# DakeQQ/Automatic-Speech-Recognition-ASR-ONNX

Measured on AMD Instinct MI355X. Metric: audio-sec/s, SenseVoiceSmall, 8 s @ 16 kHz chunks, batch 64 per GPU (RTF = 1/value per GPU-stream), higher is better.
Workload: dtype bf16; 1 GPU; SenseVoiceSmall bf16 (234 M params, 70 SANM blocks), batch=64 x 8 s per GPU, greedy CTC; step k's audio is resident in HBM when the step starts, batch k+1's host->device copy (pinned, copy stream) and every token-id download are inside the timed region; global_batch=64, parallelism=dp1 (utterance sharding, RCCL arena broadcast + hypothesis gather)

## Files before the change

### automatic-speech-recognition-asr-onnx_amd/_probe.py

```python
from __future__ import annotations

import ctypes as C
import os

import numpy as np

from . import _lib

PROBE_PATH = os.path.join(os.path.dirname(os.path.abspath(__file__)), "libasr_mi355x_probe.so")
_fp, _ip = C.POINTER(C.c_float), C.POINTER(C.c_int32)


class GemmDesc(C.Structure):
    _fields_ = [("M", C.c_int32), ("N", C.c_int32), ("K", C.c_int32), ("a", _fp), ("w", _fp), ("bias", _fp), ("add", _fp),
                ("act", C.c_int32), ("ln", C.c_int32), ("ln_eps", C.c_float), ("argmax", C.c_int32), ("n_valid", C.c_int32),
                ("variant", C.c_int32), ("out_lo", _fp), ("out_f32", _fp), ("out_stats", _fp), ("out_ids", _ip),
                ("kernel", C.c_char * 32)]


class DecodeAttnDesc(C.Structure):
    _fields_ = [("bf16", C.c_int32), ("cross", C.c_int32), ("B", C.c_int32), ("b0", C.c_int32), ("nb", C.c_int32), ("H", C.c_int32),
                ("n", C.c_int32), ("causal", C.c_int32), ("q", _fp), ("ld_q", C.c_int32), ("q_col0", C.c_int32), ("max_keys", C.c_int32),
                ("kv_new", _fp), ("k_hist", _fp), ("v_hist", _fp), ("hist", C.c_int32), ("hist_dev", C.c_int32), ("max_pos", C.c_int32),
                ("paged", C.c_int32), ("n_pages", C.c_int32), ("pages_per_seq", C.c_int32), ("page_table", _ip), ("k_after", _fp), ("v_after", _fp),
                ("k_slab", _fp), ("v_slab", _fp), ("rows", C.c_int32), ("row_off", _ip), ("n_lfr", _ip), ("fp8", C.c_int32),
                ("kv8", C.c_void_p), ("scale8", _fp), ("out", _fp), ("stray", C.c_int32), ("kernel", C.c_char * 32)]


class QwenAttnDesc(C.Structure):
    _fields_ = [("bf16", C.c_int32), ("step", C.c_int32), ("no_fuse", C.c_int32), ("B", C.c_int32), ("H", C.c_int32), ("KV", C.c_int32),
                ("rows", C.c_int32), ("qkv", _fp), ("qn", _fp), ("kn", _fp), ("rope", _fp), ("rope_rows", C.c_int32), ("eps", C.c_float),
                ("hist", _ip), ("T", _ip), ("row_off", _ip), ("row_seq", _ip), ("row_t", _ip), ("S_max", C.c_int32), ("paged", C.c_int32),
                ("n_pages", C.c_int32), ("pps", C.c_int32), ("table", _ip), ("hist_ld", C.c_int32), ("k_hist", _fp), ("v_hist", _fp),
                ("after_ld", C.c_int32), ("k_after", _fp), ("v_after", _fp), ("beam", C.c_int32), ("ld_src", C.c_int32), ("S_hyp", C.c_int32),
                ("src", _ip), ("p0", _ip), ("ext_k", _fp), ("ext_v", _fp), ("q_out", _fp), ("k_rows_out", _fp), ("ctx", _fp),
                ("stray", C.c_int32), ("qt", C.c_int32), ("nw", C.c_int32), ("kernel", C.c_char * 32)]


class BeamSelectDesc(C.Structure):
    _fields_ = [("n_utt", C.c_int32), ("beam", C.c_int32), ("K", C.c_int32), ("ld", C.c_int32), ("first", C.c_int32), ("n_slots", C.c_int32),
                ("n_stop", C.c_int32), ("topv", _fp), ("topi", _ip), ("cum", _fp), ("fin", _ip), ("len", _ip), ("next", _ip), ("done", _ip),
                ("stop", _ip), ("src_in", _ip), ("tok_in", _ip), ("src_out", _ip), ("tok_out", _ip)]


class TokenHeadDesc(C.Structure):
    _fields_ = [("op", C.c_int32), ("rows", C.c_int32), ("n_valid", C.c_int32), ("ld", C.c_int32), ("logits", _fp), ("vec", _fp),
                ("K", C.c_int32), ("ld_save", C.c_int32), ("n_saved", C.c_int32), ("n_saved_after", C.c_int32), ("save_ids", _ip),
                ("range", C.c_int32), ("partial", C.c_int32), ("value", C.c_float), ("next_in", _ip),
                ("temperature", C.c_float), ("top_p", C.c_float), ("repetition_penalty", C.c_float), ("noise", _fp), ("seed", C.c_uint64),
                ("no_speech_id", C.c_int32), ("out_v", _fp), ("out_i", _ip),
                ("steps", C.c_int32), ("track_history", C.c_int32), ("sampling", C.c_int32), ("change_step", C.c_int32), ("range2", C.c_int32),
                ("value2", C.c_float), ("picks", _ip)]


SIGNATURES = {
    "asr_probe_gemm": (C.c_int, [C.POINTER(GemmDesc)]),
    "asr_probe_ctc_head": (C.c_int, [C.c_int] * 3 + [_fp, _fp, _fp, C.c_int, C.c_int, _ip, _fp, _ip, C.c_char_p]),
    "asr_probe_gemm_chain": (C.c_int, [C.c_int] * 6 + [_fp]),
    "asr_probe_last_kernel": (C.c_char_p, []),
    "asr_probe_quantize_fp8": (C.c_int, [C.c_void_p, C.c_int, C.c_int, C.c_void_p, _fp, C.c_void_p]),
    "asr_probe_quantize_mxfp4": (C.c_int, [C.c_void_p, C.c_int, C.c_int, C.c_void_p, C.c_void_p, C.c_void_p]),
    "asr_probe_decode_gemm_mxfp4": (C.c_int, [C.c_int, C.c_int, C.c_int, C.c_void_p, C.c_void_p, C.c_void_p, C.c_void_p, _fp, C.c_int, _fp]),
    "asr_probe_decode_gemm": (C.c_int, [C.c_int, C.c_int, C.c_int, C.c_void_p, C.c_void_p, C.c_void_p, _fp, _fp, C.c_int, _fp]),
    "asr_probe_decode_attention": (C.c_int, [C.POINTER(DecodeAttnDesc)]),
    "asr_probe_qwen_attention": (C.c_int, [C.POINTER(QwenAttnDesc)]),
    "asr_probe_beam_select": (C.c_int, [C.POINTER(BeamSelectDesc)]),
    "asr_probe_token_head": (C.c_int, [C.POINTER(TokenHeadDesc)]),
    "asr_probe_decode_attention_beam": (C.c_int, [C.c_int] * 8 + [_ip, C.c_int, _fp, _fp, _fp, _fp, _ip, C.c_char_p]),
    "asr_probe_gemm_counts": (C.c_int, [C.c_int, C.c_char_p, C.c_int]),
    "asr_probe_live_device_bytes": (C.c_int, [C.POINTER(C.c_int64)]),
    "asr_probe_gemm_fp8": (C.c_int, [C.c_int, C.c_int, C.c_int, C.c_void_p, C.c_void_p, _fp, C.c_float, _fp, _fp, C.c_int, C.c_void_p, _fp, C.c_int, _fp]),
    "asr_probe_gemm_bench": (C.c_int, [C.c_int] * 6 + [_fp]),
    "asr_probe_grid_barrier": (C.c_int, [C.c_int, C.c_int, _fp]),
    "asr_probe_grid_barrier2": (C.c_int, [C.c_int, C.c_int, C.c_int, _fp]),
}
_plib = None


def load():
    global _plib
    if _plib is None:
        _lib.load()
        if not os.path.isfile(PROBE_PATH):
            raise ImportError(f"{PROBE_PATH} is missing: run `python -c 'import __graft_entry__ as g; g.build()'`")
        lib = C.CDLL(PROBE_PATH)
        for name, (res, args) in SIGNATURES.items():
            fn = getattr(lib, name)
            fn.restype, fn.argtypes = res, args
        _plib = lib
    return _plib


def _f32(a):
    return np.ascontiguousarray(a, dtype=np.float32)


def gemm(a, w, bias=None, add=None, act=0, ln=False, ln_eps=1e-5, argmax=False, n_valid=0, variant=-1, want=("lo",)):
    a, w = _f32(a), _f32(w)
    M, K = a.shape
    N = w.shape[0]
    d = GemmDesc()
    d.M, d.N, d.K, d.act, d.ln, d.ln_eps, d.argmax, d.n_valid, d.variant = M, N, K, act, int(ln), ln_eps, int(argmax), n_valid, variant
    keep = [a, w]
    d.a, d.w = a.ctypes.data_as(_fp), w.ctypes.data_as(_fp)
    if bias is not None:
        bias = _f32(bias); keep.append(bias); d.bias = bias.ctypes.data_as(_fp)
    if add is not None:
        add = _f32(add); keep.append(add); d.add = add.ctypes.data_as(_fp)
    out = {}
    if argmax:
        out["ids"] = np.zeros((M,), dtype=np.int32); d.out_ids = out["ids"].ctypes.data_as(_ip)
    else:
        if "lo" in want:
            out["lo"] = np.zeros((M, N), dtype=np.float32); d.out_lo = out["lo"].ctypes.data_as(_fp)
        if "f32" in want:
            out["f32"] = np.zeros((M, N), dtype=np.float32); d.out_f32 = out["f32"].ctypes.data_as(_fp)
        if "stats" in want:
            out["stats"] = np.zeros((M, N // 32, 2), dtype=np.float32); d.out_stats = out["stats"].ctypes.data_as(_fp)
    _lib.check(load().asr_probe_gemm(C.byref(d)))
    return out, d.kernel.decode()


def ctc_head(a, w, bias, n_valid=0, variant=-1):
    a, w, bias = _f32(a), _f32(w), _f32(bias)
    M, K = a.shape
    N = w.shape[0]
    ids, lp = np.zeros((M,), dtype=np.int32), np.zeros((M,), dtype=np.float32)
    stray, name = C.c_int32(-1), C.create_string_buffer(32)
    _lib.check(load().asr_probe_ctc_head(M, N, K, a.ctypes.data_as(_fp), w.ctypes.data_as(_fp), bias.ctypes.data_as(_fp), n_valid, variant,
                                         ids.ctypes.data_as(_ip), lp.ctypes.data_as(_fp), C.byref(stray), name))
    return ids, lp, stray.value, name.value.decode()


def gemm_bench(M, N, K, variant=-1, epilogue=0, iters=50) -> float:
    ms = C.c_float(0.0)
    _lib.check(load().asr_probe_gemm_bench(variant, M, N, K, epilogue, iters, C.byref(ms)))
    return ms.value


def gemm_set_variant(variant: int = -1) -> None:
    gemm_bench(1152, 256, 64, variant, 0, 1)


def gemm_counts(reset: bool = False) -> dict:
    buf = C.create_string_buffer(1024)
    _lib.check(load().asr_probe_gemm_counts(int(reset), buf, 1024))
    return {k: int(v) for k, v in (kv.split("=") for kv in buf.value.decode().split(";") if kv)}


def live_device_bytes() -> int:
    n = C.c_int64(0)
    _lib.check(load().asr_probe_live_device_bytes(C.byref(n)))
    return n.value


def gemm_chain(M, N, K, epilogue=0, cold_mb=768, replays=5):
    us = C.c_float(0.0)
    _lib.check(load().asr_probe_gemm_chain(M, N, K, epilogue, cold_mb, replays, C.byref(us)))
    return us.value, load().asr_probe_last_kernel().decode()


def decode_attention(q, bf16=True, n=1, B=None, b0=0, nb=0, ld_q=None, q_col0=0, max_keys=0,
                     kv_new=None, k_hist=None, v_hist=None, causal=True, hist_dev=False, max_pos=0, page_table=None, n_pages=0,
                     k_slab=None, v_slab=None, row_off=None, n_lfr=None, fp8=False):
    q = _f32(q)
    d = DecodeAttnDesc()
    cross = k_slab is not None
    H = (k_slab.shape[0] if cross else kv_new.shape[1] // 128)
    if B is None:
        B = (len(n_lfr) if cross else k_hist.shape[0])
    d.bf16, d.cross, d.B, d.b0, d.nb, d.H, d.n = int(bf16), int(cross), B, b0, nb, H, n
    d.causal = int(causal and not cross)
    d.ld_q, d.q_col0, d.max_keys = (ld_q or q.shape[1]), q_col0, max_keys
    assert q.shape == (B * n, d.ld_q), q.shape
    keep = [q]
    d.q = q.ctypes.data_as(_fp)
    out = np.zeros((B * n, H * 64), np.float32)
    d.out = out.ctypes.data_as(_fp)
    after = None
    if not cross:
        kv_new, k_hist, v_hist = _f32(kv_new), _f32(k_hist), _f32(v_hist)
        hist = k_hist.shape[2]
        assert kv_new.shape == (B * n, 2 * H * 64) and k_hist.shape == v_hist.shape == (B, H, hist, 64)
        keep += [kv_new, k_hist, v_hist]
        d.kv_new, d.k_hist, d.v_hist = kv_new.ctypes.data_as(_fp), k_hist.ctypes.data_as(_fp), v_hist.ctypes.data_as(_fp)
        d.hist, d.hist_dev, d.max_pos = hist, int(hist_dev), max_pos
        if page_table is not None:
            pt = np.ascontiguousarray(page_table, np.int32)
            keep.append(pt)
            d.paged, d.n_pages, d.pages_per_seq, d.page_table = 1, n_pages, pt.shape[1], pt.ctypes.data_as(_ip)
# ... 261 lines not shown
```

### automatic-speech-recognition-asr-onnx_amd/csrc/gemm_dev.h

```cpp
#pragma once
#include "gemm.h"

namespace {

enum { E_ADD = 1, E_ADD2 = 2, E_F32 = 4, E_LO = 8, E_AMAX = 32, E_BIAS = 64, E_LN = 128, E_ST = 256, E_LSE = 512 };

template <int ACT>
__device__ __forceinline__ float apply_act_ct(float v) {
  if constexpr (ACT == ACT_RELU) return fmaxf(v, 0.0f);
  else if constexpr (ACT == ACT_GELU_ERF) return 0.5f * v * (1.0f + erff(v * 0.70710678118654752440f));
  else if constexpr (ACT == ACT_GELU_TANH) {
    const float u = 0.7978845608028654f * (v + 0.044715f * v * v * v);
    return 0.5f * v * (1.0f + tanhf(u));
  } else return v;
}

typedef float f32pair_t __attribute__((ext_vector_type(2)));
__device__ __forceinline__ void gelu_erf_fast2(float& v0, float& v1) {
  const f32pair_t a = {fminf(fabsf(v0), 12.0f), fminf(fabsf(v1), 12.0f)};
  f32pair_t q = a * 3.30953373e-05f + -0.000769241955f;
  q = q * a + 0.00808078996f;
  q = q * a + -0.0534122179f;
  q = q * a + -0.458770889f;
  q = q * a + -1.15120173f;
// ... 2 lines not shown
  v1 = fmaf(-a.y, __builtin_amdgcn_exp2f(q.y), fmaxf(v1, 0.0f));
}
__device__ __forceinline__ float gelu_erf_fast(float v) {
  float w = v;
  gelu_erf_fast2(v, w);
  return v;
}

__device__ __forceinline__ float apply_act_rt(float v, int act) {
  switch (act) {
    case ACT_RELU: return apply_act_ct<ACT_RELU>(v);
    case ACT_GELU_ERF: return apply_act_ct<ACT_GELU_ERF>(v);
    case ACT_GELU_TANH: return apply_act_ct<ACT_GELU_TANH>(v);
    default: return v;
  }
}

__device__ __forceinline__ int xcd_remap(int bid, int nwg) {
  const int q = nwg >> 3, r = nwg & 7;
  const int xcd = bid & 7, idx = bid >> 3;
  const int base = (xcd < r) ? xcd * (q + 1) : r * (q + 1) + (xcd - r) * q;
  return base + idx;
}

__device__ __forceinline__ int frag_col(int j, int fr) { return (j >> 1) * 32 + ((fr >> 2) << 3) + ((j & 1) << 2) + (fr & 3); }
__device__ __forceinline__ int w_swz(int r) { return (((r >> 3) & 3) << 1) | ((r >> 1) & 1); }

template <int EPI, int F> __device__ __forceinline__ bool epi_has(const void* p) {
  if constexpr (EPI < 0) return p != nullptr; else return (EPI & F) != 0;
}

template <typename OutT> __device__ __forceinline__ void store4(OutT* p, float a, float b, float c, float d);
template <> __device__ __forceinline__ void store4<float>(float* p, float a, float b, float c, float d) {
  *reinterpret_cast<float4*>(p) = make_float4(a, b, c, d);
}
template <> __device__ __forceinline__ void store4<bf16_t>(bf16_t* p, float a, float b, float c, float d) {
  uint2 w;
  w.x = pack_bf16x2(a, b);
  w.y = pack_bf16x2(c, d);
  *reinterpret_cast<uint2*>(p) = w;
}

template <typename OutT> __device__ __forceinline__ void store8(OutT* p, const float (&v)[8]);
template <> __device__ __forceinline__ void store8<float>(float* p, const float (&v)[8]) {
  *reinterpret_cast<float4*>(p) = make_float4(v[0], v[1], v[2], v[3]);
  *reinterpret_cast<float4*>(p + 4) = make_float4(v[4], v[5], v[6], v[7]);
}
template <> __device__ __forceinline__ void store8<bf16_t>(bf16_t* p, const float (&v)[8]) {
  uint4 w;
  w.x = pack_bf16x2(v[0], v[1]); w.y = pack_bf16x2(v[2], v[3]); w.z = pack_bf16x2(v[4], v[5]); w.w = pack_bf16x2(v[6], v[7]);
  *reinterpret_cast<uint4*>(p) = w;
}

template <typename OutT, int ACT, int EPI, int NJ, int MI = 4>
__device__ __forceinline__ void epilogue_rows(const GemmArgs& g, f32x4_t (&acc)[MI][NJ], int m_wave, int n_wave, int lane,
                                              const float2* ln_stats = nullptr,
                                              const float* bias_at = nullptr) {
  static_assert(NJ % 2 == 0, "fragments are paired");
  const int frow = lane & 15, fgrp = lane >> 4;
  const bool has_bias = epi_has<EPI, E_BIAS>(g.bias), has_add = epi_has<EPI, E_ADD>(g.add), has_add2 = epi_has<EPI, E_ADD2>(g.add2);
  const bool want_f32 = epi_has<EPI, E_F32>(g.out_f32), want_lo = epi_has<EPI, E_LO>(g.out_lo);
  if (epi_has<EPI, E_AMAX>(g.amax_val)) {
    const int n_slabs = g.N / (NJ * 16), slab = n_wave / (NJ * 16);
#pragma unroll
    for (int i = 0; i < MI; ++i) {
      float best = -INFINITY;
      int bidx = 0x7fffffff;
#pragma unroll
      for (int j = 0; j < NJ; ++j) {
        const int n0 = n_wave + frag_col(j, fgrp * 4);
#pragma unroll
        for (int r = 0; r < 4; ++r) {
          float v = acc[i][j][r] + (has_bias ? (bias_at ? bias_at : g.bias)[n0 + r] : 0.0f);
          if (n0 + r >= g.n_valid) v = -INFINITY;
          if (v > best) { best = v; bidx = n0 + r; }
        }
      }
#pragma unroll
      for (int o = 16; o < 64; o <<= 1) {
        const float ov = __shfl_xor(best, o, 64);
        const int oi = __shfl_xor(bidx, o, 64);
        if (ov > best || (ov == best && oi < bidx)) { best = ov; bidx = oi; }
      }
      const int m = m_wave + i * 16 + frow;
      if (fgrp == 0 && m < g.M) {
        g.amax_val[(size_t)m * n_slabs + slab] = best;
        g.amax_idx[(size_t)m * n_slabs + slab] = bidx;
      }
      if ((EPI >= 0 || NJ == 4) && epi_has<EPI, E_LSE>(g.amax_sum)) {
        float sum = 0.0f;
        if (best != -INFINITY) {
#pragma unroll
          for (int j = 0; j < NJ; ++j) {
            const int n0 = n_wave + frag_col(j, fgrp * 4);
#pragma unroll
            for (int r = 0; r < 4; ++r) {
              float v = acc[i][j][r] + (has_bias ? (bias_at ? bias_at : g.bias)[n0 + r] : 0.0f);
              if (n0 + r >= g.n_valid) v = -INFINITY;
              sum += __expf(v - best);
            }
          }
        }
        sum += __shfl_xor(sum, 16, 64);
        sum += __shfl_xor(sum, 32, 64);
        if (fgrp == 0 && m < g.M) g.amax_sum[(size_t)m * n_slabs + slab] = sum;
      }
    }
  }
  if (!(want_f32 || want_lo)) return;
#pragma unroll
  for (int p = 0; p < NJ / 2; ++p) {
    const int n = n_wave + p * 32 + fgrp * 8;
    float b8[8] = {0.f, 0.f, 0.f, 0.f, 0.f, 0.f, 0.f, 0.f};
    if (has_bias) {
      const float* bp = bias_at ? bias_at : g.bias;
      const float4 lo = *reinterpret_cast<const float4*>(bp + n), hi = *reinterpret_cast<const float4*>(bp + n + 4);
      b8[0] = lo.x; b8[1] = lo.y; b8[2] = lo.z; b8[3] = lo.w; b8[4] = hi.x; b8[5] = hi.y; b8[6] = hi.z; b8[7] = hi.w;
    }
    float c8[8] = {0.f, 0.f, 0.f, 0.f, 0.f, 0.f, 0.f, 0.f};
    if constexpr (EPI >= 0 && (EPI & E_LN) != 0) {
      const float4 lo = *reinterpret_cast<const float4*>(g.ln_colsum + n), hi = *reinterpret_cast<const float4*>(g.ln_colsum + n + 4);
      c8[0] = lo.x; c8[1] = lo.y; c8[2] = lo.z; c8[3] = lo.w; c8[4] = hi.x; c8[5] = hi.y; c8[6] = hi.z; c8[7] = hi.w;
    }
    float4 t1[MI][2], t2[MI][2];
    if (has_add) {
#pragma unroll
      for (int i = 0; i < MI; ++i) {
        const float* q = g.add + (size_t)min(m_wave + i * 16 + frow, g.M - 1) * g.ld_add + n;
        t1[i][0] = *reinterpret_cast<const float4*>(q);
        t1[i][1] = *reinterpret_cast<const float4*>(q + 4);
      }
    }
    if (has_add2) {
#pragma unroll
      for (int i = 0; i < MI; ++i) {
        const int m = min(m_wave + i * 16 + frow, g.M - 1);
        const float* q = g.add2 + (size_t)(g.add2_rows ? g.add2_rows[m] : m) * g.ld_add2 + n;
        t2[i][0] = *reinterpret_cast<const float4*>(q);
        t2[i][1] = *reinterpret_cast<const float4*>(q + 4);
      }
    }
#pragma unroll
    for (int i = 0; i < MI; ++i) {
      const int m = m_wave + i * 16 + frow;
      float v[8];
#pragma unroll
      for (int r = 0; r < 4; ++r) { v[r] = acc[i][2 * p][r]; v[4 + r] = acc[i][2 * p + 1][r]; }
      if constexpr (EPI >= 0 && (EPI & E_LN) != 0) {
        const float2 mr = ln_stats[i * 16 + frow];
#pragma unroll
        for (int e = 0; e < 8; ++e) v[e] = (v[e] - mr.x * c8[e]) * mr.y;
      }
#pragma unroll
      for (int e = 0; e < 8; ++e) v[e] += b8[e];
// ... 200 lines not shown
```

### automatic-speech-recognition-asr-onnx_amd/csrc/kernels.h

```cpp
#pragma once
#include "common.h"

struct UttPlan {
  int64_t audio_off;
  int32_t n_samples;
  int32_t n_frames;
  int32_t frame_off;
  int32_t n_lfr;
  int32_t T;
  int32_t row_off;
  int32_t lang;
  int32_t blk0;
};

enum { AUDIO_F32 = 0, AUDIO_I16 = 1, AUDIO_F16 = 2 };
inline size_t audio_elt_bytes(int audio_dtype) { return audio_dtype == AUDIO_F32 ? 4 : 2; }
struct FbankArgs {
  const void* audio;
  const UttPlan* plan;
  const int32_t* blk_utt;
  const int32_t* blk_f0;
  const float* dft_packed;
  const float* mel_packed;
  float* mel_out;
  int n_bin_tiles;
  int n_kchunks;
  int n_mel_tiles;
  int n_mels;
  int win, hop;
  float log_floor;
  int whisper;
  int dbg = 0;
  float* blk_max;
  const void* dft_split = nullptr;
  int audio_dtype = AUDIO_F32;
};
void launch_fbank(const FbankArgs& a, int n_blocks, hipStream_t s);
size_t fbank_split_table_bytes(int n_bin_tiles, int win);
void launch_fbank_split_table(const float* dft_packed, int n_bin_tiles, int n_kchunks16, void* out, hipStream_t s);

template <typename T>
void launch_whisper_mel_finish(const float* mel, const float* blk_max, const UttPlan* plan, const int32_t* grow_utt,
                               int n_gapped_rows, int n_mels, T* out, hipStream_t s);
void launch_compact_rows(const float* src, const UttPlan* from, const UttPlan* to, const int32_t* row_utt, int rows, int d, float* dst, hipStream_t s);
template <typename T>
void launch_zero_gap_rows(T* buf, int ld, int n_cols, const UttPlan* plan, const int32_t* grow_utt, int n_gapped_rows,
                          hipStream_t s);

void launch_layernorm_fp8(const float* x, int ld_x, int rows, int D, float eps, float inv_scale, unsigned char* out, int ld_out, hipStream_t s);

template <typename T>
void launch_embed_pos(const int32_t* ids, int rows, int n, int hist, const int32_t* hist_dev, const T* embed, const float* pos, int d,
                      float* x, hipStream_t s);
void launch_add_scalar(int32_t* p, int v, hipStream_t s);

struct DecAttnArgs {
  const void* q; int ld_q; int q_col0;
  const void* kv_new; int ld_new; int k_col0, v_col0;
  void* k_base; void* v_base;
  int64_t stride_b, stride_h;
  const UttPlan* plan;
  int hist, n, n_heads, causal;
  int max_keys = 0;
  int sc_ld = 0;
  const int32_t* hist_dev;
  void* out; int ld_out;
  const float* k_scale = nullptr; const float* v_scale = nullptr;
  const int32_t* page_table = nullptr; int pages_per_seq = 0; int64_t page_stride = 0;
  int b0 = 0, scale_ld = 0;
  const int32_t* beam_src = nullptr; int ld_src = 0, beam_p0 = 0, beam = 1;
};
void launch_quantize_rows_fp8(const bf16_t* W, int ld, int N, int K, unsigned char* W8, float* scale, bf16_t* Wdq, hipStream_t s);
void launch_quantize_rows_mxfp4(const bf16_t* W, int ld, int N, int K, unsigned char* W4, unsigned char* S, bf16_t* Wdq, hipStream_t s);
void launch_quantize_crosskv_fp8(bf16_t* slabs, size_t slab_elems, int n_slabs, const UttPlan* plan, int batch, unsigned char* out8, float* scale,
                                 int dq_in_place, hipStream_t s);
template <typename T>
void launch_decode_attention(const DecAttnArgs& a, int batch, hipStream_t s);
const char* decode_attn_last_kernel();

constexpr int BEAM_MAX = 8;
void launch_beam_topk(const float* logits, int ld, int rows, int n_valid, const float* bias, int K, float* topv, int32_t* topi, hipStream_t s);
struct BeamArgs {
  int beam, K, ld, first, n_slots;
  const float* topv; const int32_t* topi;
  float* cum; int32_t* fin; int32_t* len; int32_t* next; int32_t* done;
  const int32_t* stop; int n_stop;
  const int32_t *src_in, *tok_in; int32_t *src_out, *tok_out;
  const int32_t* slots_dev = nullptr;
// ... 241 lines not shown
```

### automatic-speech-recognition-asr-onnx_amd/csrc/kernels.hip

```cpp
#include "kernels.h"
#include "gemm.h"

#include <algorithm>
#include <type_traits>
#include <cstdlib>

namespace {

constexpr int HOP = 160, WIN = 400;
constexpr int FB_FRAMES = 64;
constexpr int FB_SPAN = (FB_FRAMES - 1) * HOP + WIN;
constexpr int FB_AUDIO_LDS = FB_SPAN + FB_SPAN / HOP + 16;
constexpr int FB_PLD = 273;

template <typename S> struct Pcm;
template <> struct Pcm<float> {
  typedef float raw_t;
  static __device__ __forceinline__ raw_t load(const float* p, int i) { return p[i]; }
  static __device__ __forceinline__ raw_t hold(raw_t r) { return r; }
  static __device__ __forceinline__ float widen(raw_t r, float) { return r; }
};
template <> struct Pcm<int16_t> {
  typedef int raw_t;
  static __device__ __forceinline__ raw_t load(const int16_t* p, int i) { return p[i]; }
  static __device__ __forceinline__ raw_t hold(raw_t r) { asm volatile("" : "+v"(r)); return r; }
  static __device__ __forceinline__ float widen(raw_t r, float scale) { return (float)r * scale; }
};
template <> struct Pcm<_Float16> {
  typedef uint32_t raw_t;
  static __device__ __forceinline__ raw_t load(const _Float16* p, int i) { return reinterpret_cast<const uint16_t*>(p)[i]; }
  static __device__ __forceinline__ raw_t hold(raw_t r) { asm volatile("" : "+v"(r)); return r; }
  static __device__ __forceinline__ float widen(raw_t r, float) { return (float)__builtin_bit_cast(_Float16, (uint16_t)r); }
};

template <typename S>
__global__ __launch_bounds__(256) void fbank_kernel(const FbankArgs a) {
  extern __shared__ __attribute__((aligned(16))) unsigned char smem[];
  float* aud = reinterpret_cast<float*>(smem);
  float* pw = aud + FB_AUDIO_LDS;
  const int tid = threadIdx.x, lane = tid & 63, wave = tid >> 6;
  const int u = a.blk_utt[blockIdx.x], f0 = a.blk_f0[blockIdx.x];
  const UttPlan up = a.plan[u];
  const S* src = static_cast<const S*>(a.audio) + up.audio_off;
  const float pcm_scale = a.whisper ? 0x1p-15f : 1.0f;
  const int s0 = f0 * HOP;
  constexpr int NL = (FB_SPAN + 255) / 256;
  typename Pcm<S>::raw_t av[NL];
#pragma unroll
  for (int j = 0; j < NL; ++j) {
    const int i = tid + j * 256, L = up.n_samples, half = WIN / 2, p = s0 + i;
    int idx = p;
    bool ok = i < FB_SPAN && p < L;
    if (a.whisper) {
      idx = p < half ? half - p : p < half + L ? p - half : 2 * L + half - 2 - p;
      ok = i < FB_SPAN && p < L + WIN - HOP;
    }
    av[j] = ok ? Pcm<S>::load(src, idx) : (typename Pcm<S>::raw_t)0;
  }
#pragma unroll
  for (int j = 0; j < NL; ++j) av[j] = Pcm<S>::hold(av[j]);
#pragma unroll
  for (int j = 0; j < NL; ++j) {
    const int i = tid + j * 256;
    if (i < FB_SPAN) aud[i + i / HOP] = Pcm<S>::widen(av[j], pcm_scale);
  }
  __syncthreads();

  const int frow = lane & 15, fgrp = lane >> 4;
  const float4* dft = reinterpret_cast<const float4*>(a.dft_packed);
  for (int t = wave; t < a.n_bin_tiles; t += 4) {
    f32x4_t re[4], im[4];
#pragma unroll
    for (int mt = 0; mt < 4; ++mt) { re[mt] = f32x4_t{0.f, 0.f, 0.f, 0.f}; im[mt] = f32x4_t{0.f, 0.f, 0.f, 0.f}; }
    const float4* dre = dft + (size_t)(t * 2 + 0) * a.n_kchunks * 64 + lane;
    const float4* dim = dft + (size_t)(t * 2 + 1) * a.n_kchunks * 64 + lane;
    float4 br = dre[0], bi = dim[0];
    for (int kc = 0; kc < a.n_kchunks; ++kc) {
      float4 brn = br, bin = bi;
      if (kc + 1 < a.n_kchunks) { brn = dre[(kc + 1) * 64]; bin = dim[(kc + 1) * 64]; }
      const float brv[4] = {br.x, br.y, br.z, br.w};
      const float biv[4] = {bi.x, bi.y, bi.z, bi.w};
#pragma unroll
      for (int j = 0; j < 4; ++j) {
        const int k = kc * 16 + j * 4 + fgrp;
        const int koff = k + k / HOP;
        float af[4];
#pragma unroll
        for (int mt = 0; mt < 4; ++mt) af[mt] = aud[(mt * 16 + frow) * (HOP + 1) + koff];
#pragma unroll
        for (int mt = 0; mt < 4; ++mt) {
          re[mt] = __builtin_amdgcn_mfma_f32_16x16x4f32(af[mt], brv[j], re[mt], 0, 0, 0);
          im[mt] = __builtin_amdgcn_mfma_f32_16x16x4f32(af[mt], biv[j], im[mt], 0, 0, 0);
        }
      }
      br = brn; bi = bin;
    }
#pragma unroll
    for (int mt = 0; mt < 4; ++mt)
#pragma unroll
      for (int r = 0; r < 4; ++r)
        pw[(mt * 16 + fgrp * 4 + r) * FB_PLD + t * 16 + frow] = re[mt][r] * re[mt][r] + im[mt][r] * im[mt][r];
  }
  __syncthreads();

  float wmax = -INFINITY;
  const float4* melp = reinterpret_cast<const float4*>(a.mel_packed);
  for (int nt = 0; nt < a.n_mel_tiles; ++nt) {
    f32x4_t acc = f32x4_t{0.f, 0.f, 0.f, 0.f};
    float4 b4 = melp[(size_t)(nt * a.n_bin_tiles) * 64 + lane];
    for (int kc = 0; kc < a.n_bin_tiles; ++kc) {
      float4 b4n = b4;
      if (kc + 1 < a.n_bin_tiles) b4n = melp[(size_t)(nt * a.n_bin_tiles + kc + 1) * 64 + lane];
      const float bv[4] = {b4.x, b4.y, b4.z, b4.w};
#pragma unroll
      for (int j = 0; j < 4; ++j) {
        const float av = pw[(wave * 16 + frow) * FB_PLD + kc * 16 + j * 4 + fgrp];
        acc = __builtin_amdgcn_mfma_f32_16x16x4f32(av, bv[j], acc, 0, 0, 0);
      }
      b4 = b4n;
    }
#pragma unroll
    for (int r = 0; r < 4; ++r) {
      const int f = f0 + wave * 16 + fgrp * 4 + r;
      if (f < up.n_frames) {
        const float c = fmaxf(acc[r], a.log_floor);
        const float v = a.whisper ? log10f(c) : logf(c);
        a.mel_out[(size_t)(up.frame_off + f) * a.n_mels + nt * 16 + frow] = v;
        wmax = fmaxf(wmax, v);
      }
    }
  }
  if (a.whisper) {
    __shared__ float red[4];
    wmax = wave_max(wmax);
    if (lane == 0) red[wave] = wmax;
    __syncthreads();
    if (tid == 0) a.blk_max[blockIdx.x] = fmaxf(fmaxf(red[0], red[1]), fmaxf(red[2], red[3]));
  }
}

constexpr int FB_HP = HOP + 8;
constexpr int FB_K32 = (WIN + 31) / 32;
constexpr int FB_A16 = ((FB_SPAN + 32 + HOP - 1) / HOP) * FB_HP;

constexpr int FB_WAVES = 8;
template <typename S>
__global__ __launch_bounds__(64 * FB_WAVES) void fbank_split_kernel(const FbankArgs a) {
  extern __shared__ __attribute__((aligned(16))) unsigned char smem[];
  bf16_t* audh = reinterpret_cast<bf16_t*>(smem);
  bf16_t* audl = audh + FB_A16;
  float* pw = reinterpret_cast<float*>(audl + FB_A16);
  const int tid = threadIdx.x, lane = tid & 63, wave = tid >> 6;
  const int u = a.blk_utt[blockIdx.x], f0 = a.blk_f0[blockIdx.x];
  const UttPlan up = a.plan[u];
  const S* src = static_cast<const S*>(a.audio) + up.audio_off;
  const float pcm_scale = a.whisper ? 0x1p-15f : 1.0f;
  const int s0 = f0 * HOP;
  constexpr int FB_NL = (FB_SPAN + 32 + 64 * FB_WAVES - 1) / (64 * FB_WAVES);
  typename Pcm<S>::raw_t av[FB_NL];
#pragma unroll
  for (int j = 0; j < FB_NL; ++j) {
    const int i = tid + j * 64 * FB_WAVES;
    const int L = up.n_samples, half = WIN / 2, p = s0 + i;
    int idx = p;
    bool ok = i < FB_SPAN + 32 && p < L;
    if (a.whisper) {
      idx = p < half ? half - p : p < half + L ? p - half : 2 * L + half - 2 - p;
      ok = i < FB_SPAN + 32 && p < L + WIN - HOP;
    }
    av[j] = (ok && !(a.dbg & 4)) ? Pcm<S>::load(src, idx) : (typename Pcm<S>::raw_t)0;
  }
#pragma unroll
  for (int j = 0; j < FB_NL; ++j) av[j] = Pcm<S>::hold(av[j]);
#pragma unroll
  for (int j = 0; j < FB_NL; ++j) {
    const int i = tid + j * 64 * FB_WAVES;
    if (i < FB_SPAN + 32) {
      const float v = Pcm<S>::widen(av[j], pcm_scale);
      const uint32_t hb = pack_bf16x2(v, 0.0f) & 0xffffu;
      const float hi = __uint_as_float(hb << 16);
      const int pos = i + (i / HOP) * 8;
      audh[pos] = (bf16_t)hb;
      audl[pos] = (bf16_t)(pack_bf16x2(v - hi, 0.0f) & 0xffffu);
    }
  }
  __syncthreads();

  const int frow = lane & 15, fgrp = lane >> 4;
  const uint4* tab = reinterpret_cast<const uint4*>(a.dft_split);
  constexpr int FB_PF = 4;
  union BF { uint4 q; bf16x8_t v; };
  BF ring[FB_PF][6];
  const int wv = __builtin_amdgcn_readfirstlane(wave);
  const int n_steps = (wv < a.n_bin_tiles && !(a.dbg & 1)) ? (a.n_bin_tiles - wv + FB_WAVES - 1) / FB_WAVES * FB_K32 : 0;
  constexpr size_t FB_IM = (size_t)FB_K32 * 3 * 64;
  auto frag_ptr = [&](int t, int kc) { return tab + (((size_t)(t * 2) * FB_K32 + kc) * 3) * 64 + lane; };
  int pt = wv, pkc = 0, ps = 0;
  auto refill = [&](BF (&slot)[6]) {
    const uint4* src = frag_ptr(pt, pkc);
#pragma unroll
    for (int z = 0; z < 3; ++z) { slot[z].q = src[z * 64]; slot[3 + z].q = src[FB_IM + z * 64]; }
    if (ps + 1 < n_steps) { ++ps; if (++pkc == FB_K32) { pkc = 0; pt += FB_WAVES; } }
  };
  f32x4_t re[4], im[4];
#pragma unroll
  for (int mt = 0; mt < 4; ++mt) { re[mt] = f32x4_t{0.f, 0.f, 0.f, 0.f}; im[mt] = f32x4_t{0.f, 0.f, 0.f, 0.f}; }
  if (n_steps > 0) {
#pragma unroll
    for (int u = 0; u < FB_PF; ++u) refill(ring[u]);
  }
  int t = wv, kc = 0;
  for (int s0 = 0; s0 < n_steps; s0 += FB_PF) {
#pragma unroll
    for (int u = 0; u < FB_PF; ++u) {
      if (s0 + u < n_steps) {
        const int k = kc * 32 + fgrp * 8;
        const int koff = k + ((k >= HOP) + (k >= 2 * HOP)) * 8;
        bf16x8_t ah[4], al[4];
#pragma unroll
        for (int mt = 0; mt < 4; ++mt) {
          const int pos = (mt * 16 + frow) * FB_HP + koff;
          ah[mt] = *reinterpret_cast<const bf16x8_t*>(audh + pos); al[mt] = *reinterpret_cast<const bf16x8_t*>(audl + pos);
        }
#define ASR_FB_TERM(X, ZR, ZI)                                                                          \
        _Pragma("unroll") for (int mt = 0; mt < 4; ++mt) {                                               \
          re[mt] = __builtin_amdgcn_mfma_f32_16x16x32_bf16(X[mt], ring[u][ZR].v, re[mt], 0, 0, 0);       \
          im[mt] = __builtin_amdgcn_mfma_f32_16x16x32_bf16(X[mt], ring[u][ZI].v, im[mt], 0, 0, 0);       \
        }
        ASR_FB_TERM(al, 1, 4)
        ASR_FB_TERM(ah, 2, 5)
        ASR_FB_TERM(al, 0, 3)
        ASR_FB_TERM(ah, 1, 4)
        ASR_FB_TERM(ah, 0, 3)
#undef ASR_FB_TERM
        if (++kc == FB_K32) {
#pragma unroll
          for (int mt = 0; mt < 4; ++mt) {
#pragma unroll
            for (int r = 0; r < 4; ++r)
              pw[(mt * 16 + fgrp * 4 + r) * FB_PLD + t * 16 + frow] = re[mt][r] * re[mt][r] + im[mt][r] * im[mt][r];
            re[mt] = f32x4_t{0.f, 0.f, 0.f, 0.f}; im[mt] = f32x4_t{0.f, 0.f, 0.f, 0.f};
          }
          kc = 0; t += FB_WAVES;
        }
      }
      __builtin_amdgcn_sched_barrier(0);
      if (!(a.dbg & 8)) refill(ring[u]);
      __builtin_amdgcn_sched_barrier(0);
    }
  }
  __syncthreads();

  float wmax = -INFINITY;
  const float4* melp = reinterpret_cast<const float4*>(a.mel_packed);
  constexpr int FB_MT = 4;
  const int fw = wave & 3, mg = wave >> 2;
  for (int nt0 = mg; nt0 < ((a.dbg & 2) ? 0 : a.n_mel_tiles); nt0 += 2 * FB_MT) {
    f32x4_t acc[FB_MT];
#pragma unroll
    for (int q = 0; q < FB_MT; ++q) acc[q] = f32x4_t{0.f, 0.f, 0.f, 0.f};
    auto mel_frags = [&](float4 (&b)[FB_MT], int kc) {
#pragma unroll
      for (int q = 0; q < FB_MT; ++q) b[q] = nt0 + 2 * q < a.n_mel_tiles ? melp[(size_t)((nt0 + 2 * q) * a.n_bin_tiles + kc) * 64 + lane] : make_float4(0.f, 0.f, 0.f, 0.f);
    };
    float4 b4[FB_MT], b4n[FB_MT];
    mel_frags(b4, 0);
    for (int kc = 0; kc < a.n_bin_tiles; ++kc) {
      mel_frags(b4n, kc + 1 < a.n_bin_tiles ? kc + 1 : kc);
#pragma unroll
      for (int j = 0; j < 4; ++j) {
        const float av = pw[(fw * 16 + frow) * FB_PLD + kc * 16 + j * 4 + fgrp];
#pragma unroll
        for (int q = 0; q < FB_MT; ++q) {
          const float bv = j == 0 ? b4[q].x : j == 1 ? b4[q].y : j == 2 ? b4[q].z : b4[q].w;
          if (nt0 + 2 * q < a.n_mel_tiles) acc[q] = __builtin_amdgcn_mfma_f32_16x16x4f32(av, bv, acc[q], 0, 0, 0);
        }
      }
#pragma unroll
      for (int q = 0; q < FB_MT; ++q) b4[q] = b4n[q];
    }
#pragma unroll
    for (int q = 0; q < FB_MT; ++q) {
      if (nt0 + 2 * q >= a.n_mel_tiles) continue;
#pragma unroll
      for (int r = 0; r < 4; ++r) {
        const int f = f0 + fw * 16 + fgrp * 4 + r;
        if (f < up.n_frames) {
          const float c = fmaxf(acc[q][r], a.log_floor);
          const float v = a.whisper ? log10f(c) : logf(c);
          a.mel_out[(size_t)(up.frame_off + f) * a.n_mels + (nt0 + 2 * q) * 16 + frow] = v;
          wmax = fmaxf(wmax, v);
        }
      }
    }
  }
  if (a.whisper) {
    __shared__ float red[FB_WAVES];
    wmax = wave_max(wmax);
    if (lane == 0) red[wave] = wmax;
    __syncthreads();
    if (tid == 0) {
      float m = red[0];
#pragma unroll
      for (int w = 1; w < FB_WAVES; ++w) m = fmaxf(m, red[w]);
      a.blk_max[blockIdx.x] = m;
    }
  }
}

__global__ void fbank_split_table_kernel(const float* __restrict__ dft_packed, int n_bin_tiles, int n_kchunks16, uint4* __restrict__ out) {
  const int idx = blockIdx.x * blockDim.x + threadIdx.x;
  const int total = n_bin_tiles * 2 * FB_K32 * 64;
  if (idx >= total) return;
  const int lane = idx & 63, kc = (idx >> 6) % FB_K32, tr = (idx >> 6) / FB_K32;
  const int frow = lane & 15, fgrp = lane >> 4;
  uint32_t w[3][4] = {};
  for (int e = 0; e < 8; ++e) {
    const int k = kc * 32 + fgrp * 8 + e;
    float v = 0.0f;
    if (k < n_kchunks16 * 16) {
      v = dft_packed[(((size_t)tr * n_kchunks16 + (k >> 4)) * 64 + ((k & 3) * 16 + frow)) * 4 + ((k & 15) >> 2)];
    }
    float r = v;
    for (int z = 0; z < 3; ++z) {
      const uint32_t b = pack_bf16x2(r, 0.0f) & 0xffffu;
      r -= __uint_as_float(b << 16);
      w[z][e >> 1] |= b << ((e & 1) * 16);
    }
  }
  for (int z = 0; z < 3; ++z) out[((size_t)(tr * FB_K32 + kc) * 3 + z) * 64 + lane] = make_uint4(w[z][0], w[z][1], w[z][2], w[z][3]);
}

// ... 1070 lines not shown
        if (mm >= s && mm < e) acc = fmaf(w[c * ktaps + j], x[(size_t)mm * d + c], acc);
      }
    }
    out[(size_t)m * d + c] = acc;
  }
}

__global__ __launch_bounds__(256) void token_compact_kernel(const UttPlan* __restrict__ own, int n_utts, int n_rows_max,
                                                            UttPlan* __restrict__ compact, int32_t* __restrict__ row_utt,
                                                            int32_t* __restrict__ total_rows) {
  __shared__ int total_s;
  if (threadIdx.x == 0) {
    int off = 0;
    for (int u = 0; u < n_utts; ++u) {
      UttPlan tp = own[u];
      tp.row_off = off;
      compact[u] = tp;
      off += (tp.T + 15) & ~15;
    }
    total_s = off;
    *total_rows = off;
  }
  __syncthreads();
  const int total = total_s;
  for (int r = threadIdx.x; r < n_rows_max; r += 256) row_utt[r] = -1;
  __syncthreads();
  for (int u = 0; u < n_utts; ++u) {
    const int r0 = compact[u].row_off, n16 = (compact[u].T + 15) & ~15;
    for (int r = threadIdx.x; r < n16; r += 256)
      if (r0 + r < min(total, n_rows_max)) row_utt[r0 + r] = u;
  }
}

__global__ __launch_bounds__(256) void compact_rows_kernel(const float* __restrict__ src, const UttPlan* __restrict__ own,
                                                           const UttPlan* __restrict__ compact, int d, float* __restrict__ dst) {
  const int u = blockIdx.x, s0 = own[u].row_off, d0 = compact[u].row_off, n16 = (compact[u].T + 15) & ~15;
  for (int e = threadIdx.x; e < n16 * d; e += 256) dst[(size_t)d0 * d + e] = src[(size_t)s0 * d + e];
}

__global__ void gather_tokens_kernel(const int32_t* __restrict__ ids, const UttPlan* __restrict__ tplan, int32_t* __restrict__ token_ids,
                                     int max_tokens) {
  const int u = blockIdx.x;
  const int n = min(tplan[u].n_lfr, max_tokens);
  for (int i = threadIdx.x; i < n; i += blockDim.x) token_ids[(size_t)u * max_tokens + i] = ids[tplan[u].row_off + i];
}

}

template <typename S>
static void launch_fbank_typed(const FbankArgs& a, int n_blocks, hipStream_t s) {
  ASR_REQUIRE(a.win == WIN && a.hop == HOP, "fbank: only win=400 hop=160 is built (got %d/%d)", a.win, a.hop);
  ASR_REQUIRE(a.n_bin_tiles * 16 <= FB_PLD - 1, "fbank: too many frequency bins");
  ASR_REQUIRE(a.n_kchunks * 16 == WIN, "fbank: k-chunks must cover the window");
  const size_t lds = (size_t)(FB_AUDIO_LDS + FB_FRAMES * FB_PLD) * sizeof(float);
  static PerDeviceOnce attr_once;
  if (attr_once.first()) {
    HIP_CHECK(hipFuncSetAttribute(reinterpret_cast<const void*>(fbank_kernel<S>), hipFuncAttributeMaxDynamicSharedMemorySize, (int)lds));
  }
  if (a.dft_split) {
    FbankArgs b = a;
    if (const char* e = getenv("ASR_FBANK_DBG")) b.dbg = atoi(e);
    const size_t lds2 = (size_t)FB_A16 * 2 * 2 + (size_t)FB_FRAMES * FB_PLD * sizeof(float);
    static PerDeviceOnce attr2_once;
    if (attr2_once.first()) {
      HIP_CHECK(hipFuncSetAttribute(reinterpret_cast<const void*>(fbank_split_kernel<S>), hipFuncAttributeMaxDynamicSharedMemorySize, (int)lds2));
    }
    hipLaunchKernelGGL(fbank_split_kernel<S>, dim3(n_blocks), dim3(64 * FB_WAVES), lds2, s, b);
    HIP_CHECK(hipGetLastError());
    return;
  }
  hipLaunchKernelGGL(fbank_kernel<S>, dim3(n_blocks), dim3(256), lds, s, a);
  HIP_CHECK(hipGetLastError());
}
void launch_fbank(const FbankArgs& a, int n_blocks, hipStream_t s) {
  switch (a.audio_dtype) {
    case AUDIO_F32: return launch_fbank_typed<float>(a, n_blocks, s);
    case AUDIO_I16: return launch_fbank_typed<int16_t>(a, n_blocks, s);
    case AUDIO_F16: return launch_fbank_typed<_Float16>(a, n_blocks, s);
    default: ASR_THROW(ASR_ERR_INVALID, "fbank: unknown audio sample type %d", a.audio_dtype);
  }
}

size_t fbank_split_table_bytes(int n_bin_tiles, int win) {
  ASR_REQUIRE(win == WIN, "fbank: only win=400 is built (got %d)", win);
  return (size_t)n_bin_tiles * 2 * FB_K32 * 3 * 64 * 16;
}
void launch_fbank_split_table(const float* dft_packed, int n_bin_tiles, int n_kchunks16, void* out, hipStream_t s) {
  const int total = n_bin_tiles * 2 * FB_K32 * 64;
  hipLaunchKernelGGL(fbank_split_table_kernel, dim3((total + 255) / 256), dim3(256), 0, s, dft_packed, n_bin_tiles, n_kchunks16, reinterpret_cast<uint4*>(out));
  HIP_CHECK(hipGetLastError());
}

void launch_lfr_cmvn(const LfrArgs& a, hipStream_t s) {
  hipLaunchKernelGGL(lfr_cmvn_kernel, dim3(a.n_rows), dim3(256), 0, s, a);
  HIP_CHECK(hipGetLastError());
}

template <typename OutT>
void launch_layernorm(const float* x, int ld_x, int rows, int D, const float* gamma, const float* beta, float eps,
                      OutT* out, int ld_out, int fill_to, hipStream_t s, const int32_t* rows_dev) {
  ASR_REQUIRE(D % 4 == 0 && D <= LN_MAXV * 256 && ld_x % 4 == 0 && ld_out % 4 == 0, "layernorm: D=%d ld=%d unsupported", D, ld_x);
  hipLaunchKernelGGL(layernorm_kernel<OutT>, dim3((rows + 3) / 4), dim3(256), 0, s, x, ld_x, rows, D, gamma, beta, eps, out,
                     ld_out, fill_to, rows_dev, (bf16_t*)nullptr, 0);
  HIP_CHECK(hipGetLastError());
}
void launch_layernorm_with_bf16_copy(const float* x, int ld_x, int rows, int D, const float* gamma, const float* beta, float eps,
                                     float* out, int ld_out, bf16_t* out_lo, int ld_lo, hipStream_t s) {
  ASR_REQUIRE(D % 4 == 0 && D <= LN_MAXV * 256 && ld_x % 4 == 0 && ld_out % 4 == 0 && ld_lo % 4 == 0 && out_lo, "layernorm: D=%d ld=%d unsupported", D, ld_x);
  hipLaunchKernelGGL(layernorm_kernel<float>, dim3((rows + 3) / 4), dim3(256), 0, s, x, ld_x, rows, D, gamma, beta, eps, out, ld_out, D, (const int32_t*)nullptr, out_lo, ld_lo);
  HIP_CHECK(hipGetLastError());
}
template void launch_layernorm<float>(const float*, int, int, int, const float*, const float*, float, float*, int, int, hipStream_t, const int32_t*);
template void launch_layernorm<bf16_t>(const float*, int, int, int, const float*, const float*, float, bf16_t*, int, int, hipStream_t, const int32_t*);

void launch_layernorm_fp8(const float* x, int ld_x, int rows, int D, float eps, float inv_scale, unsigned char* out, int ld_out, hipStream_t s) {
  ASR_REQUIRE(D % 256 == 0 && D <= 2048 && ld_x % 4 == 0 && ld_out % 4 == 0, "layernorm_fp8: D=%d unsupported", D);
  hipLaunchKernelGGL(layernorm_fp8_kernel, dim3((rows + 3) / 4), dim3(256), 0, s, x, ld_x, rows, D, eps, inv_scale, out, ld_out);
  HIP_CHECK(hipGetLastError());
}

template <int HD, int CHUNK, int QT>
static void launch_attn_inst(const AttnArgs& a, hipStream_t s) {
  constexpr int lds = CHUNK * HD * 2 * 2;
  static PerDeviceOnce attr_once;
  if (attr_once.first()) {
    HIP_CHECK(hipFuncSetAttribute(reinterpret_cast<const void*>(attn_bf16_kernel<HD, CHUNK, QT>),
                                  hipFuncAttributeMaxDynamicSharedMemorySize, lds));
  }
  AttnArgs b = a;
  if (b.ld_q == 0) b.ld_q = b.ld_qk;
  hipLaunchKernelGGL((attn_bf16_kernel<HD, CHUNK, QT>), dim3(a.n_qblocks, a.n_heads), dim3(64 * a.n_waves), lds, s, b, a.ld_vt);
  HIP_CHECK(hipGetLastError());
}
// ... 1117 lines not shown
```

### automatic-speech-recognition-asr-onnx_amd/csrc/probe.hip

```cpp
#include <algorithm>
#include <cmath>
#include <cstring>
#include <vector>

#include "../../include/asr_mi355x.h"
#include "../../include/asr_mi355x_probe.h"
#include "decode_head.h"
#include "engine.h"
#include "gemm.h"
#include "kernels.h"
#include "qwen_attn.h"

namespace {

struct Tmp {
  std::vector<void*> ptrs;
  ~Tmp() { for (void* p : ptrs) (void)hipFree(p); }
  void* alloc(size_t bytes) {
    void* p = nullptr;
    HIP_CHECK(hipMalloc(&p, std::max<size_t>(bytes, 256)));
    HIP_CHECK(hipMemset(p, 0, std::max<size_t>(bytes, 256)));
    ptrs.push_back(p);
    return p;
  }
};

inline int round_up(int v, int m) { return (v + m - 1) / m * m; }
char g_chain_kernel[32] = "";
inline float bf16_bits_to_f32(bf16_t b) { union { uint32_t u; float f; } c; c.u = ((uint32_t)b) << 16; return c.f; }

}

extern "C" int asr_probe_gemm_bench(int variant, int M, int N, int K, int epilogue, int iters, float* avg_ms) {
  return asr_guard([&] {
    ASR_REQUIRE(avg_ms && iters > 0, "probe_gemm_bench: bad argument");
    asr_require_device(0);
    Tmp t;
    const int Mp = round_up(M, 128);
    auto rnd = [](size_t n, uint32_t seed) {
      std::vector<bf16_t> v(n);
      uint32_t x = seed;
      for (size_t i = 0; i < n; ++i) { x = x * 1664525u + 1013904223u; v[i] = f32_to_bf16(((int)(x >> 9) % 2001 - 1000) * 1e-3f); }
      return v;
    };
    std::vector<bf16_t> ha = rnd((size_t)Mp * K, 1), hw = rnd((size_t)N * K, 2);
    bf16_t* da = (bf16_t*)t.alloc(ha.size() * 2);
    bf16_t* dw = (bf16_t*)t.alloc(hw.size() * 2);
    HIP_CHECK(hipMemcpy(da, ha.data(), ha.size() * 2, hipMemcpyHostToDevice));
    HIP_CHECK(hipMemcpy(dw, hw.data(), hw.size() * 2, hipMemcpyHostToDevice));
    float* bias = (float*)t.alloc((size_t)N * 4);
    float* addm = (float*)t.alloc((size_t)Mp * N * 4);
    float* addt = (float*)t.alloc((size_t)Mp * N * 4);
    float* of32 = (float*)t.alloc((size_t)Mp * N * 4);
    bf16_t* olo = (bf16_t*)t.alloc((size_t)Mp * N * 2);
    bf16_t* ot = (bf16_t*)t.alloc((size_t)Mp * N * 2);
    GemmArgs g;
    g.A = da; g.lda = K; g.W = dw; g.ldw = K; g.M = M; g.N = N; g.K = K; g.bias = bias;
    switch (epilogue) {
      case 0: g.out_lo = olo; g.ld_out_lo = N; break;
      case 1: g.out_lo = olo; g.ld_out_lo = N; g.act = ACT_RELU; break;
      case 2: g.add = addm; g.ld_add = N; g.out_f32 = of32; g.ld_out_f32 = N; break;
      case 7: g.out_lo = olo; g.ld_out_lo = N; g.act = ACT_GELU_ERF; break;
      case 3: g.bias = nullptr; g.add = addt; g.ld_add = N; g.add2 = addm; g.ld_add2 = N; g.out_f32 = of32; g.ld_out_f32 = N; break;
      case 4: g.out_t = ot; g.ld_out_t = Mp; break;
      case 5: {
        float2* st = (float2*)t.alloc((size_t)Mp * (K / 32) * 8);
        HIP_CHECK(hipMemset(st, 0, (size_t)Mp * (K / 32) * 8));
        g.out_lo = olo; g.ld_out_lo = N; g.act = ACT_RELU; g.ln_colsum = bias; g.ln_dim = K; g.ln_stats_in = st; g.ln_slots = K / 32;
        break;
      }
      case 6: {
        float2* st = (float2*)t.alloc((size_t)Mp * (N / 32) * 8);
        g.bias = nullptr; g.add = addt; g.ld_add = N; g.add2 = addm; g.ld_add2 = N; g.out_f32 = of32; g.ld_out_f32 = N;
        g.out_lo = olo; g.ld_out_lo = N; g.st_out = st;
        break;
      }
      default: ASR_THROW(ASR_ERR_INVALID, "probe_gemm_bench: unknown epilogue %d", epilogue);
    }
    g.dbg = variant < 0 ? 0 : variant >> 8;
    uint32_t* clk = nullptr;
    if (getenv("ASR_PP_CLK")) { clk = (uint32_t*)t.alloc(64 * 4); HIP_CHECK(hipMemset(clk, 0, 64 * 4)); g.dbg_clk = clk; }
    gemm_set_variant(variant < 0 ? -1 : (variant & 0xff));
    hipEvent_t e0, e1;
    HIP_CHECK(hipEventCreate(&e0));
    HIP_CHECK(hipEventCreate(&e1));
    for (int i = 0; i < 3; ++i) launch_gemm_bf16(g, nullptr);
    HIP_CHECK(hipEventRecord(e0, nullptr));
    for (int i = 0; i < iters; ++i) launch_gemm_bf16(g, nullptr);
    HIP_CHECK(hipEventRecord(e1, nullptr));
    HIP_CHECK(hipEventSynchronize(e1));
    float ms = 0.f;
    HIP_CHECK(hipEventElapsedTime(&ms, e0, e1));
    *avg_ms = ms / iters;
    if (clk) {
      uint32_t h[40];
      HIP_CHECK(hipMemcpy(h, clk, sizeof(h), hipMemcpyDeviceToHost));
      const int ksteps = K / 64 - 2;
      for (int w = 0; w < 2; ++w)
        for (int r = 0; r < 4; ++r)
          fprintf(stderr, "pp clock: group %d phase %d: reads %6.1f  vmcnt %6.1f  barrier %6.1f | mfma %6.1f  barrier %6.1f  (cycles per phase)\n", w, r,
                  h[w * 20 + r * 5] / (double)ksteps, h[w * 20 + r * 5 + 1] / (double)ksteps, h[w * 20 + r * 5 + 2] / (double)ksteps,
                  h[w * 20 + r * 5 + 3] / (double)ksteps, h[w * 20 + r * 5 + 4] / (double)ksteps);
    }
    gemm_set_variant(-1);
    (void)hipEventDestroy(e0);
    (void)hipEventDestroy(e1);
  });
}


extern "C" int asr_probe_gemm_chain(int M, int N, int K, int epilogue, int cold_mb, int replays, float* us_per_launch) {
  return asr_guard([&] {
    ASR_REQUIRE(us_per_launch && replays > 0 && M > 0 && N % 16 == 0 && K % 256 == 0, "probe_gemm_chain: bad argument");
    asr_require_device(0);
    gemm_reload_env();
    Tmp t;
    const int Mp = round_up(M, 128);
    const size_t wbytes = (size_t)N * K * 2;
    const int copies = std::max(1, std::min(512, (int)(((size_t)cold_mb << 20) / wbytes) + 1));
    std::vector<bf16_t> hw((size_t)N * K), ha((size_t)Mp * K);
    uint32_t x = 12345;
    for (auto& v : hw) { x = x * 1664525u + 1013904223u; v = f32_to_bf16(((int)(x >> 9) % 2001 - 1000) * 1e-3f); }
    for (auto& v : ha) { x = x * 1664525u + 1013904223u; v = f32_to_bf16(((int)(x >> 9) % 2001 - 1000) * 1e-3f); }
    bf16_t* dw = (bf16_t*)t.alloc(wbytes * copies);
    for (int c = 0; c < copies; ++c) HIP_CHECK(hipMemcpy((char*)dw + wbytes * c, hw.data(), wbytes, hipMemcpyHostToDevice));
    bf16_t* da = (bf16_t*)t.alloc(ha.size() * 2);
    HIP_CHECK(hipMemcpy(da, ha.data(), ha.size() * 2, hipMemcpyHostToDevice));
    float* bias = (float*)t.alloc((size_t)N * 4);
    float* addm = (float*)t.alloc((size_t)Mp * N * 4);
    float* of32 = (float*)t.alloc((size_t)Mp * N * 4);
    bf16_t* olo = (bf16_t*)t.alloc((size_t)Mp * N * 2);
    float* lnx = (float*)t.alloc((size_t)Mp * K * 4);
    GemmArgs g;
    g.A = da; g.lda = K; g.ldw = K; g.M = M; g.N = N; g.K = K; g.bias = bias;
    g.sk_ws = (float*)t.alloc((size_t)16 << 20); g.sk_ws_bytes = (size_t)16 << 20; g.sk_cnt = (int32_t*)t.alloc(4096 * 4);
    switch (epilogue >= 10 ? 0 : epilogue) {
      case 0: g.out_lo = olo; g.ld_out_lo = N; break;
      case 1: g.out_lo = olo; g.ld_out_lo = N; g.act = ACT_GELU_ERF; break;
      case 2: g.add = addm; g.ld_add = N; g.out_f32 = of32; g.ld_out_f32 = N; break;
      case 3: g.A = nullptr; g.ln_x = lnx; g.ld_ln_x = K; g.out_lo = olo; g.ld_out_lo = N; break;
      default: ASR_THROW(ASR_ERR_INVALID, "probe_gemm_chain: unknown epilogue %d", epilogue);
    }
    hipStream_t s;
    HIP_CHECK(hipStreamCreate(&s));
    const int chain = std::max(copies, 64);
    DecGemmArgs dg;
    const bool use_dg = epilogue >= 10;
    if (use_dg) {
      const int e = epilogue - 10;
      float* cs = (float*)t.alloc((size_t)N * 4);
      dg.A = da; dg.lda = K; dg.ldw = K; dg.M = M; dg.N = N; dg.K = K; dg.bias = bias;
      dg.ws = g.sk_ws; dg.ws_bytes = g.sk_ws_bytes; dg.cnt = g.sk_cnt;
      if (e == 0) { dg.out_lo = olo; dg.ld_out_lo = N; }
      else if (e == 1) { dg.out_lo = olo; dg.ld_out_lo = N; dg.act = ACT_GELU_ERF; dg.colsum = cs; }
      else if (e == 2) { dg.add = addm; dg.ld_add = N; dg.out_f32 = of32; dg.ld_out_f32 = N; dg.out_lo = olo; dg.ld_out_lo = N; }
      else if (e == 3) { dg.out_lo = olo; dg.ld_out_lo = N; dg.colsum = cs; }
      else ASR_THROW(ASR_ERR_INVALID, "probe_gemm_chain: unknown decode epilogue %d", e);
      int nt = 1, sp = 1;
      decode_gemm_plan(dg, &nt, &sp);
      snprintf(g_chain_kernel, sizeof(g_chain_kernel), "decode nt%d ks%d", nt, sp);
    }
    const bool prefetch = use_dg && getenv("ASR_PROBE_PREFETCH") && getenv("ASR_PROBE_PREFETCH")[0] == '1';
// ... 1028 lines not shown
```

### automatic-speech-recognition-asr-onnx_amd/csrc/qwen.hip

```cpp
#include <cstdlib>
#include <cstring>
#include <type_traits>
#include <vector>

#include "../../include/asr_mi355x.h"
#include "decode_head.h"
#include "engine.h"
#include "gemm.h"
#include "kernels.h"
#include "qwen_attn.h"

namespace {

inline int round_up(int v, int m) { return (v + m - 1) / m * m; }

inline int feat_lengths(int n) {
  const int leave = n % 100;
  const int f1 = leave > 0 ? (std::max(leave - 1, 0) / 2 + 1) : 0;
  const int f2 = f1 > 0 ? (std::max(f1 - 1, 0) / 2 + 1) : 0;
  const int f3 = f2 > 0 ? (std::max(f2 - 1, 0) / 2 + 1) : 0;
  return f3 + (n / 100) * 13;
}

inline size_t pad_rows(size_t r) { return (r + 127) / 128 * 128 + 144; }
// ... 505 lines not shown
}

__global__ __launch_bounds__(256) void qw_slot_compact_kernel(const int32_t* __restrict__ src, const UttPlan* __restrict__ plan, int tid,
                                                              const int32_t* __restrict__ cnt, int B, int cap, int32_t* __restrict__ off,
                                                              int32_t* __restrict__ rows) {
  __shared__ int base_sh, wave_n[4];
  const int b = blockIdx.x, lane = threadIdx.x & 63, wave = threadIdx.x >> 6;
  if (threadIdx.x == 0) base_sh = 0;
  __syncthreads();
  int s = 0;
  for (int i = threadIdx.x; i < b; i += 256) s += cnt[i];
  atomicAdd(&base_sh, s);
  __syncthreads();
  int base = base_sh;
  if (threadIdx.x == 0) { off[b] = base; if (b == B - 1) off[B] = base + cnt[b]; }
  const UttPlan p = plan[b];
  for (int t0 = 0; t0 < p.T; t0 += 256) {
    const int t = t0 + threadIdx.x;
    const bool hit = t < p.T && qw_slot_hit(src, p.row_off + t, tid);
    const unsigned long long m = __ballot(hit);
    if (lane == 0) wave_n[wave] = __popcll(m);
    __syncthreads();
    int before = 0;
    for (int w = 0; w < wave; ++w) before += wave_n[w];
    const int at = base + before + __popcll(m & ((1ull << lane) - 1ull));
    if (hit && at < cap) rows[at] = p.row_off + t;
    base += wave_n[0] + wave_n[1] + wave_n[2] + wave_n[3];
    __syncthreads();
  }
}

__global__ void qw_beam_init_kernel(const int32_t* __restrict__ hist_in, int B, int beam, int32_t* __restrict__ hist_out, int32_t* __restrict__ p0) {
  const int n = blockIdx.x * blockDim.x + threadIdx.x;
  if (n < B * beam) { hist_out[n] = hist_in[n / beam]; p0[n] = hist_in[n / beam]; }
}

struct QwEncLayer { const void *wqkv, *wo, *w1, *w2; const float *bqkv, *bo, *b1, *b2; };
struct QwDecLayer { const void *wqkv, *wo, *gate_up, *down; const float *qn, *kn; };
struct QwDec8Layer { const unsigned char* w[4]; const float* s[4]; const unsigned char* s4[4]; };

struct DecPass {
  const UttPlan* plan = nullptr; const int32_t *row_seq = nullptr, *row_t = nullptr, *last_rows = nullptr;
  int rows = 0, B = 0; bool step = false, hist_done = false;
  const int32_t *qb_utt = nullptr, *qb_q0 = nullptr; int n_qb = 0, qt = 0, nw = 0, max_T = 0, ld_vt = 0;
  void *kc = nullptr, *vc = nullptr; int S = 0; int32_t* hist = nullptr; const int32_t *beam_src = nullptr, *beam_p0 = nullptr; int ld_src = 0, beam = 1;
  bool head = true;
};

struct AlignReq { int32_t tid = -1; int32_t* slot_off = nullptr; int32_t* buckets = nullptr; int64_t cap = 0; float* logits = nullptr; };

struct QwSession : asr_session {
  asr_qwen_config cfg;
  int vpad = 0, hpad = 0, cpad = 0, n_bin_tiles = 0, n_kchunks = 0, chunk = 0, cpw = 0, rpw = 0, t_tok = 13;
  std::vector<QwEncLayer> enc;
  std::vector<QwDecLayer> dec;
  const float *dft = nullptr, *melp = nullptr, *conv1_b = nullptr, *conv2_b = nullptr, *conv3_b = nullptr, *enc_pos = nullptr,
              *proj1_b = nullptr, *proj2_b = nullptr, *rope = nullptr, *final_norm = nullptr;
  const void *conv1_w = nullptr, *conv2_w = nullptr, *conv3_w = nullptr, *conv_out_w = nullptr, *proj1_w = nullptr, *proj2_w = nullptr,
             *embed = nullptr, *lm_head = nullptr;
  int batch = 0;
  std::vector<int> seq_len;
  DeviceBuffer d_plan, d_audio, d_mel, d_blkmax, d_feat, d_col, d_c1, d_c2, d_c3, d_xa, d_xb, d_h, d_qk, d_vt, d_ctx, d_ffn, d_aud_out;
  std::vector<char> frozen;
  DeviceBuffer d_dplan, d_x, d_x2, d_dh, d_qkv, d_q, d_dctx, d_act, d_last, d_logits, d_next, d_kc, d_vc, d_hist, d_stepplan, d_skws, d_skcnt, d_vt2, d_krows, d_xlo, d_x2lo;
  bool no_fuse = false, use_graph = true;
  bool fp4 = false;
  bool fp8 = false, fp8_fake = false;
  bool use_decode_gemm = true;
  std::vector<QwDec8Layer> dec8;
  DeviceBuffer d_w8, d_wscale, d_wdq;
  bool kv_paged = true, kv_shuffle = false;
  int kv_pps = 0, kv_pool_pages = 0, kv_high_water = 0;
  std::vector<int32_t> kv_free, kv_table;
  std::vector<std::vector<int32_t>> kv_owned;
  std::vector<char> kv_released;
  DeviceBuffer d_kvtab;
  PinnedBuffer h_kvtab;
  bool kv_table_dirty = false;
  size_t kv_page_elems() const { return (size_t)cfg.n_layers * cfg.n_kv_heads * 16 * cfg.d_head; }
  void kv_begin(int B, const std::vector<int>& lens, size_t eT);
  void kv_prepare_step(size_t eT);
  int kv_take(size_t eT);
  void kv_upload();
  KvAddr kv_addr() const {
    if (kv_paged) return KvAddr{d_kvtab.as<int32_t>(), kv_pps, kv_page_elems(), cfg.max_seq_len};
    return KvAddr{nullptr, 0, 0, cfg.max_seq_len};
  }
  TokenHead head;
  DeviceBuffer d_sel, d_amax_v, d_amax_i, d_bucket;
  DeviceBuffer d_bkc, d_bvc, d_bhist, d_bp0, d_bplan;
  BeamRanker ranker;
  StepGraph dec_graph;
  PinnedBuffer h_plan, h_io, h_ids;

  void gemm(const GemmArgs& g0) {
    if (precision != ASR_PRECISION_BF16) { launch_gemm_f32(g0, stream); return; }
    if (!d_skws.ptr) { d_skws.reserve((size_t)16 << 20, stream); d_skcnt.reserve(4096 * 4, stream); }
    GemmArgs g = g0;
    g.sk_ws = d_skws.as<float>(); g.sk_ws_bytes = d_skws.cap; g.sk_cnt = d_skcnt.as<int32_t>();
    launch_gemm_bf16(g, stream);
  }
  void init();
  bool aligner() const { return cfg.classify_num > 0; }
  template <typename T> void prefill(const void* audio, int audio_mem, const int64_t* offs, int B, const int32_t* pre_ids, const int32_t* pre_off,
                                     const int32_t* post_ids, const int32_t* post_off, int32_t* next_out, float* logits_out, int32_t* ids_len_out,
                                     const AlignReq* al = nullptr);
  template <typename T> void align_head(int B, const UttPlan* ddp, const int32_t* d_src, int n_sel, const AlignReq& al);
  template <typename T> void decoder_pass(const DecPass& P);
  template <typename T> void logits_head(const DecPass& P);
  template <typename T> void step(const int32_t* ids_host, int32_t* next_out, float* logits_out);
  void finish(int B, int32_t* next_out, float* logits_out, bool sync);
  template <typename T> void beam_search(int beam, int max_new, const int32_t* stop_ids, int n_stop, int32_t* tokens_out, int32_t* n_out, float* scores_out);
};

void QwSession::init() {
  const auto& c = cfg;
  ASR_REQUIRE(c.nfft == 400 && c.hop_length == 160 && c.n_mels == 128, "qwen: front-end is built for n_fft 400 / hop 160 / 128 mels");
  ASR_REQUIRE(c.d_head == 128 && c.n_heads % c.n_kv_heads == 0, "qwen: decoder head_dim must be 128");
  ASR_REQUIRE(c.enc_d % 128 == 0 && c.enc_d / c.enc_heads == 64 && c.enc_ffn % 128 == 0, "qwen: encoder needs 64-wide heads and widths that are multiples of 128");
  ASR_REQUIRE(c.d_model % 128 == 0 && c.d_ffn % 64 == 0 && (2 * c.d_ffn) % 128 == 0, "qwen: decoder widths must be multiples of 128");
  ASR_REQUIRE(c.n_window == 50, "qwen: the conv stem is built for 100-frame chunks (n_window 50)");
  chunk = 2 * c.n_window;
  cpw = c.n_window_infer / chunk;
  rpw = round_up(cpw * t_tok, 16);
  ASR_REQUIRE(cpw >= 1 && rpw <= 1024, "qwen: bad attention window");
  vpad = round_up(c.vocab, 128);
  head.init(c.max_seq_len, 1, 10, 1024);
  ASR_REQUIRE(c.classify_num >= 0, "qwen: classify_num %d", c.classify_num);
  hpad = aligner() ? round_up(c.classify_num, 128) : vpad;
  cpad = round_up(c.conv_channels, 128);
  n_bin_tiles = (c.nfft / 2 + 1 + 15) / 16;
  n_kchunks = c.nfft / 16;
  const int wt = precision == ASR_PRECISION_BF16 ? ARENA_BF16 : ARENA_F32;
  const int de = c.enc_d, d = c.d_model, qkvn = (c.n_heads + 2 * c.n_kv_heads) * c.d_head;
  auto F = [&](const std::string& n, std::initializer_list<int64_t> sh) { return (const float*)arena.get(n, ARENA_F32, sh).ptr; };
  auto W = [&](const std::string& n, std::initializer_list<int64_t> sh) { return arena.get(n, wt, sh).ptr; };
  dft = F("fe.dft", {(int64_t)n_bin_tiles * 2 * n_kchunks * 64 * 4});
  melp = F("fe.mel", {(int64_t)(c.n_mels / 16) * n_bin_tiles * 64 * 4});
  conv1_w = W("enc.conv1_w", {cpad, 64});          conv1_b = F("enc.conv1_b", {cpad});
  conv2_w = W("enc.conv2_w", {cpad, 9 * cpad});    conv2_b = F("enc.conv2_b", {cpad});
  conv3_w = W("enc.conv3_w", {cpad, 9 * cpad});    conv3_b = F("enc.conv3_b", {cpad});
  conv_out_w = W("enc.conv_out_w", {de, 16 * cpad});
  enc_pos = F("enc.pos", {t_tok, de});
  enc.resize(c.n_enc_layers);
  for (int i = 0; i < c.n_enc_layers; ++i) {
    const std::string q = "enc" + std::to_string(i) + ".";
    enc[i] = {W(q + "wqkv", {3 * de, de}), W(q + "wo", {de, de}), W(q + "w1", {c.enc_ffn, de}), W(q + "w2", {de, c.enc_ffn}),
              F(q + "bqkv", {3 * de}), F(q + "bo", {de}), F(q + "b1", {c.enc_ffn}), F(q + "b2", {de})};
  }
  proj1_w = W("enc.proj1_w", {de, de});   proj1_b = F("enc.proj1_b", {de});
  proj2_w = W("enc.proj2_w", {d, de});    proj2_b = F("enc.proj2_b", {d});
  embed = W("dec.embed", {vpad, d});
  lm_head = W("dec.lm_head", {hpad, d});
  rope = F("dec.rope", {c.max_seq_len, c.d_head});
  final_norm = F("dec.final_norm", {d});
  dec.resize(c.n_layers);
  for (int i = 0; i < c.n_layers; ++i) {
    const std::string q = "dec" + std::to_string(i) + ".";
    dec[i] = {W(q + "wqkv", {qkvn, d}), W(q + "wo", {d, c.n_heads * c.d_head}), W(q + "gate_up", {2 * c.d_ffn, d}), W(q + "down", {d, c.d_ffn}),
              F(q + "qn", {c.d_head}), F(q + "kn", {c.d_head})};
  }
  if (fp8) {
    const int I = c.d_ffn, od = c.n_heads * c.d_head;
    ASR_REQUIRE(d % 256 == 0 && I % 256 == 0 && od % 256 == 0, "qwen: FP8 mode needs d_model, d_ffn and heads x head_dim to be multiples of 256");
    const int Ns[4] = {qkvn, d, 2 * I, d}, Ks[4] = {d, od, d, I};
    size_t w_elems = 0, n_scales = 0;
    for (int j = 0; j < 4; ++j) { w_elems += (size_t)Ns[j] * Ks[j]; n_scales += Ns[j]; }
    d_w8.reserve(fp4 ? c.n_layers * w_elems / 2 : c.n_layers * w_elems, stream); d_wscale.reserve(fp4 ? c.n_layers * w_elems / 32 : c.n_layers * n_scales * 4, stream);
    d_wdq.reserve(c.n_layers * w_elems * 2, stream);
    dec8.resize(c.n_layers);
    for (int i = 0; i < c.n_layers; ++i) {
      QwDecLayer& L = dec[i];
      const void** slot[4] = {&L.wqkv, &L.wo, &L.gate_up, &L.down};
      unsigned char* w8 = d_w8.as<unsigned char>() + (fp4 ? i * w_elems / 2 : i * w_elems);
      bf16_t* dq = d_wdq.as<bf16_t>() + i * w_elems;
      float* sc = d_wscale.as<float>() + i * n_scales;
      unsigned char* sc4 = d_wscale.as<unsigned char>() + i * w_elems / 32;
      for (int j = 0; j < 4; ++j) {
        const size_t ne = (size_t)Ns[j] * Ks[j];
        if (fp4) launch_quantize_rows_mxfp4((const bf16_t*)*slot[j], Ks[j], Ns[j], Ks[j], w8, sc4, dq, stream);
        else launch_quantize_rows_fp8((const bf16_t*)*slot[j], Ks[j], Ns[j], Ks[j], w8, sc, dq, stream);
        dec8[i].w[j] = w8; dec8[i].s[j] = sc; dec8[i].s4[j] = sc4;
        *slot[j] = dq;
        w8 += fp4 ? ne / 2 : ne; dq += ne; sc += Ns[j]; sc4 += ne / 32;
      }
    }
    HIP_CHECK(hipStreamSynchronize(stream));
  }
}

void QwSession::kv_upload() {
// ... 332 lines not shown
      UttPlan& p = h_dp[b];
      p = up[b];
      p.T = ids_len[b]; p.n_lfr = ids_len[b]; p.row_off = drow0[b];
    }
  }
  d_plan.reserve(plan_bytes, stream);
  HIP_CHECK(hipMemcpyAsync(d_plan.ptr, hp, plan_bytes, hipMemcpyHostToDevice, stream));
  const UttPlan* dup = d_plan.as<UttPlan>();
  const UttPlan* dwp = dup + B;
  const UttPlan* ddp = dwp + wins;
  const int32_t* d_blk_utt = (const int32_t*)(ddp + B);
  const int32_t* d_blk_f0 = d_blk_utt + n_fb;
  const int32_t* d_qb_utt = d_blk_f0 + n_fb;
  const int32_t* d_qb_q0 = d_qb_utt + n_qb;
  const int32_t* d_slot_utt = d_qb_q0 + n_qb;
  const int32_t* d_slot_local = d_slot_utt + slots;
  const int32_t* d_pos_rows = d_slot_local + slots;
  const int32_t* d_src = d_pos_rows + Me;
  const int32_t* d_row_seq = d_src + Md;
  const int32_t* d_row_t = d_row_seq + Md;
  const int32_t* d_last_rows = d_row_t + Md;
  const int32_t* d_dqb_utt = d_last_rows + B;
  const int32_t* d_dqb_q0 = d_dqb_utt + n_dqb;

  const size_t eA = audio_elt();
  const void* d_aud = static_cast<const unsigned char*>(audio) + (size_t)base0 * eA;
  const int64_t total_samples = offs[B] - base0;
  if (audio_mem == ASR_MEM_HOST) {
    d_audio.reserve((size_t)total_samples * eA, stream);
    HIP_CHECK(hipMemcpyAsync(d_audio.ptr, d_aud, (size_t)total_samples * eA, hipMemcpyHostToDevice, stream));
    d_aud = d_audio.ptr;
  }
  const size_t r1 = (size_t)slots * 50 * 64, r2 = (size_t)slots * 25 * 32, r3 = (size_t)wins * rpw * 16;
  d_mel.reserve((size_t)frames * c.n_mels * 4, stream);
  d_blkmax.reserve((size_t)n_fb * 4, stream);
  d_feat.reserve((size_t)slots * chunk * c.n_mels * eT, stream);
  d_col.reserve(std::max(std::max(pad_rows(r1) * 64, pad_rows(r2) * 9 * cpad), pad_rows(r3) * 9 * cpad) * eT, stream);
  d_c1.reserve(pad_rows(r1) * cpad * eT, stream);
  d_c2.reserve(pad_rows(r2) * cpad * eT, stream);
  d_c3.reserve((r3 + 16 * 288) * cpad * eT, stream);
  d_xa.reserve((size_t)Me * de * 4, stream);
  d_xb.reserve((size_t)Me * de * 4, stream);
  d_h.reserve((size_t)Me * de * eT, stream);
  d_qk.reserve((size_t)Me * 2 * de * eT, stream);
  d_vt.reserve((size_t)Me * de * eT, stream);
  d_ctx.reserve((size_t)Me * de * eT, stream);
  d_ffn.reserve((size_t)Me * dff * eT, stream);
  d_aud_out.reserve((size_t)Me * d * 4, stream);
  {
    ProfScope ps(prof, "logmel", stream);
    FbankArgs fa;
    fa.audio = d_aud; fa.audio_dtype = audio_dtype; fa.plan = dup; fa.blk_utt = d_blk_utt; fa.blk_f0 = d_blk_f0; fa.dft_packed = dft; fa.mel_packed = melp;
    fa.mel_out = d_mel.as<float>(); fa.n_bin_tiles = n_bin_tiles; fa.n_kchunks = n_kchunks; fa.n_mel_tiles = c.n_mels / 16; fa.n_mels = c.n_mels;
    fa.win = c.nfft; fa.hop = c.hop_length; fa.log_floor = 1e-10f; fa.whisper = 1; fa.blk_max = d_blkmax.as<float>();
    launch_fbank(fa, n_fb, stream);
    if (taps_enabled) save_tap("mel", d_mel.ptr, frames, c.n_mels, c.n_mels, 4);
    hipLaunchKernelGGL(qw_mel_finish_kernel<T>, dim3(slots * chunk), dim3(128), 0, stream, d_mel.as<float>(), d_blkmax.as<float>(), dup, d_slot_utt,
                       d_slot_local, c.n_mels, chunk, d_feat.as<T>());
  }
  {
    ProfScope ps(prof, "conv_stem", stream);
    T* col = d_col.as<T>();
    hipLaunchKernelGGL(qw_im2col1_kernel<T>, dim3((unsigned)(r1 / 4)), dim3(256), 0, stream, d_feat.as<T>(), c.n_mels, chunk, 50, 64, col);
    GemmArgs g1; g1.A = col; g1.lda = 64; g1.W = conv1_w; g1.ldw = 64; g1.M = (int)r1; g1.N = cpad; g1.K = 64; g1.bias = conv1_b; g1.act = ACT_GELU_TANH;
    g1.out_lo = d_c1.ptr; g1.ld_out_lo = cpad; gemm(g1);
    hipLaunchKernelGGL(qw_im2col_cl_kernel<T>, dim3((unsigned)r2), dim3(256), 0, stream, d_c1.as<T>(), cpad, 50, 64, 25, 32, 0, 0, 0, col);
    GemmArgs g2; g2.A = col; g2.lda = 9 * cpad; g2.W = conv2_w; g2.ldw = 9 * cpad; g2.M = (int)r2; g2.N = cpad; g2.K = 9 * cpad; g2.bias = conv2_b;
    g2.act = ACT_GELU_TANH; g2.out_lo = d_c2.ptr; g2.ld_out_lo = cpad; gemm(g2);
    hipLaunchKernelGGL(qw_im2col_cl_kernel<T>, dim3((unsigned)r3), dim3(256), 0, stream, d_c2.as<T>(), cpad, 25, 32, 13, 16, rpw, cpw, t_tok, col);
    GemmArgs g3; g3.A = col; g3.lda = 9 * cpad; g3.W = conv3_w; g3.ldw = 9 * cpad; g3.M = (int)r3; g3.N = cpad; g3.K = 9 * cpad; g3.bias = conv3_b;
    g3.act = ACT_GELU_TANH; g3.out_lo = d_c3.ptr; g3.ld_out_lo = cpad; gemm(g3);
    GemmArgs g4; g4.A = d_c3.ptr; g4.lda = 16 * cpad; g4.W = conv_out_w; g4.ldw = 16 * cpad; g4.M = rows_e; g4.N = de; g4.K = 16 * cpad;
    g4.add2 = enc_pos; g4.ld_add2 = de; g4.add2_rows = d_pos_rows; g4.out_f32 = d_xa.as<float>(); g4.ld_out_f32 = de; gemm(g4);
  }
  if (taps_enabled) save_tap("stem", d_xa.ptr, rows_e, de, de, 4);
  float* xa = d_xa.as<float>();
  float* xb = d_xb.as<float>();
  T* h = d_h.as<T>();
  T* qk = d_qk.as<T>();
  T* vt = d_vt.as<T>();
  T* ctx = d_ctx.as<T>();
  T* ffn = d_ffn.as<T>();
  for (int i = 0; i < c.n_enc_layers; ++i) {
    const QwEncLayer& L = enc[i];
    { ProfScope ps(prof, "layernorm", stream); launch_layernorm<T>(xa, de, rows_e, de, nullptr, nullptr, 1e-5f, h, de, de, stream); }
    { ProfScope ps(prof, "gemm_qkv", stream);
      GemmArgs g; g.A = h; g.lda = de; g.W = L.wqkv; g.ldw = de; g.M = rows_e; g.N = 2 * de; g.K = de; g.bias = L.bqkv; g.out_lo = qk; g.ld_out_lo = 2 * de; gemm(g);
      GemmArgs gv; gv.A = h; gv.lda = de; gv.W = (const T*)L.wqkv + (size_t)2 * de * de; gv.ldw = de; gv.M = rows_e; gv.N = de; gv.K = de;
      gv.bias = L.bqkv + 2 * de; gv.out_t = vt; gv.ld_out_t = Me; gemm(gv); }
    { ProfScope ps(prof, "attention", stream);
      AttnArgs aa; aa.q = qk; aa.k = qk + de; aa.ld_qk = 2 * de; aa.vt = vt; aa.ld_vt = Me; aa.ctx = ctx; aa.ld_ctx = de; aa.plan = dwp;
      aa.qb_utt = d_qb_utt; aa.qb_q0 = d_qb_q0; aa.n_qblocks = n_qb; aa.n_heads = H; aa.qt = att_qt; aa.n_waves = att_nw; aa.max_T = max_T;
      if (precision == ASR_PRECISION_BF16) launch_attention_bf16_hd64(aa, stream); else launch_attention_f32(aa, 64, stream); }
    { ProfScope ps(prof, "gemm_out", stream);
      GemmArgs g; g.A = ctx; g.lda = de; g.W = L.wo; g.ldw = de; g.M = rows_e; g.N = de; g.K = de; g.bias = L.bo; g.add = xa; g.ld_add = de;
      g.out_f32 = xb; g.ld_out_f32 = de; gemm(g); }
    { ProfScope ps(prof, "layernorm", stream); launch_layernorm<T>(xb, de, rows_e, de, nullptr, nullptr, 1e-5f, h, de, de, stream); }
    { ProfScope ps(prof, "gemm_ffn1", stream);
      GemmArgs g; g.A = h; g.lda = de; g.W = L.w1; g.ldw = de; g.M = rows_e; g.N = dff; g.K = de; g.bias = L.b1; g.act = ACT_GELU_TANH; g.out_lo = ffn;
      g.ld_out_lo = dff; gemm(g); }
    { ProfScope ps(prof, "gemm_ffn2", stream);
      GemmArgs g; g.A = ffn; g.lda = dff; g.W = L.w2; g.ldw = dff; g.M = rows_e; g.N = de; g.K = dff; g.bias = L.b2; g.add = xb; g.ld_add = de;
      g.out_f32 = xa; g.ld_out_f32 = de; gemm(g); }
  }
  { ProfScope ps(prof, "proj", stream);
    launch_layernorm<T>(xa, de, rows_e, de, nullptr, nullptr, 1e-5f, h, de, de, stream);
    GemmArgs g; g.A = h; g.lda = de; g.W = proj1_w; g.ldw = de; g.M = rows_e; g.N = de; g.K = de; g.bias = proj1_b; g.act = ACT_GELU_TANH; g.out_lo = ctx;
// ... 191 lines not shown
    std::vector<unsigned char> blob(sbytes);
    UttPlan* sp = (UttPlan*)blob.data();
    int32_t* s_seq = (int32_t*)(sp + N); int32_t* s_t = s_seq + Mb; int32_t* s_last = s_t + Mb;
    for (int r = 0; r < Mb; ++r) { s_seq[r] = r < N ? r : -1; s_t[r] = 0; s_last[r] = r < N ? r : 0; }
    for (int n = 0; n < N; ++n) { UttPlan p{}; p.T = 1; p.n_lfr = 1; p.row_off = n; sp[n] = p; }
    d_bplan.reserve(sbytes, stream);
    HIP_CHECK(hipMemcpyAsync(d_bplan.ptr, blob.data(), sbytes, hipMemcpyHostToDevice, stream));
    HIP_CHECK(hipStreamSynchronize(stream));
  }
  const UttPlan* dsp = d_bplan.as<UttPlan>();
  DecPass P;
  P.plan = dsp; P.row_seq = (const int32_t*)(dsp + N); P.row_t = P.row_seq + Mb; P.last_rows = P.row_t + Mb; P.rows = N; P.B = N; P.step = true;
  P.kc = d_bkc.ptr; P.vc = d_bvc.ptr; P.S = Sb; P.hist = d_bhist.as<int32_t>(); P.beam_p0 = d_bp0.as<int32_t>(); P.ld_src = ld; P.beam = beam;
  for (int t = 0; t + 1 < max_new && !ranker.all_done(stream); ++t) {
    { ProfScope ps(prof, "dec_embed", stream);
      hipLaunchKernelGGL(qw_gather_prompt_kernel<T>, dim3(N), dim3(256), 0, stream, (const int32_t*)ranker.next_ids(), (const T*)embed, (const float*)nullptr, d,
                         INT32_MIN, d_x.as<float>(), precision == ASR_PRECISION_BF16 ? d_xlo.as<T>() : (T*)nullptr); }
    P.beam_src = ranker.ancestry();
    decoder_pass<T>(P);
    { ProfScope ps(prof, "beam_rank", stream);
      ranker.enqueue_rank(d_logits.as<float>(), vpad, c.vocab, t + 1, stream); }
    ranker.flip();
  }
  HIP_CHECK(hipGetLastError());
  ranker.download(tokens_out, out_stride, n_out, scores_out, stream);
  if (prof.enabled) prof.collect();
}

}

extern "C" int asr_qwen_create(const asr_qwen_config* cfg, const void* arena, size_t arena_bytes, int arena_mem, int device_id, int precision,
                               asr_session** out) {
  return asr_guard([&] {
    ASR_REQUIRE(cfg && arena && out, "qwen_create: null argument");
    ASR_REQUIRE(precision == ASR_PRECISION_BF16 || precision == ASR_PRECISION_F32 || precision == ASR_PRECISION_FP8W || precision == ASR_PRECISION_MXFP4W, "qwen_create: bad precision %d", precision);
    asr_require_device(device_id);
    QwSession* s = new QwSession();
    try {
      s->kind = 5;
      s->device = device_id;
      asr_tenant_attach(s);
      s->fp4 = precision == ASR_PRECISION_MXFP4W;
      s->fp8 = precision == ASR_PRECISION_FP8W || s->fp4;
      s->precision = s->fp8 ? ASR_PRECISION_BF16 : precision;
      s->cfg = *cfg;
      ASR_REQUIRE(cfg->classify_num == 0 || !s->fp8, "qwen_create: the forced aligner runs bf16 or f32 weights (FP8W / MXFP4W aligner sessions are not supported)");
      HIP_CHECK(hipStreamCreateWithFlags(&s->stream, hipStreamNonBlocking));
      s->own_stream = true;
      gemm_reload_env();
      if (const char* e = getenv("ASR_FP8_FAKE")) s->fp8_fake = e[0] == '1';
      if (const char* e = getenv("ASR_QWEN_DECODE_GEMM")) s->use_decode_gemm = !(e[0] == '0');
      if (const char* e = getenv("ASR_NO_GRAPH")) s->use_graph = !(e[0] == '1');
      if (const char* e = getenv("ASR_QWEN_NO_FUSE")) s->no_fuse = e[0] == '1';
      if (const char* e = getenv("ASR_QWEN_KV_PAGED")) s->kv_paged = !(e[0] == '0');
      if (const char* e = getenv("ASR_KV_PAGE_SHUFFLE")) s->kv_shuffle = e[0] == '1';
      s->arena.load(arena, arena_bytes, arena_mem, s->stream);
      s->init();
    } catch (...) {
      delete s;
      throw;
    }
    *out = s;
  });
}

extern "C" int asr_qwen_prefill(asr_session* s, const void* audio, int audio_mem, const int64_t* audio_offsets, int batch, const int32_t* pre_ids,
                                const int32_t* pre_offsets, const int32_t* post_ids, const int32_t* post_offsets, int32_t* next_ids_out,
                                float* logits_out, int32_t* ids_len_out) {
  return asr_guard([&] {
    ASR_REQUIRE(s && s->kind == 5, "qwen_prefill: not a Qwen3-ASR session");
    TenantScope tenant(s);
    QwSession* q = static_cast<QwSession*>(s);
    ASR_REQUIRE(!q->aligner(), "qwen_prefill: a forced-aligner session (classify_num %d) has no LM head; call asr_qwen_align", q->cfg.classify_num);
    if (q->precision == ASR_PRECISION_BF16)
      q->prefill<bf16_t>(audio, audio_mem, audio_offsets, batch, pre_ids, pre_offsets, post_ids, post_offsets, next_ids_out, logits_out, ids_len_out);
    else
      q->prefill<float>(audio, audio_mem, audio_offsets, batch, pre_ids, pre_offsets, post_ids, post_offsets, next_ids_out, logits_out, ids_len_out);
  });
}

extern "C" int asr_qwen_decode(asr_session* s, const int32_t* ids, int32_t* next_ids_out, float* logits_out) {
  return asr_guard([&] {
    ASR_REQUIRE(s && s->kind == 5, "qwen_decode: not a Qwen3-ASR session");
    TenantScope tenant(s);
    QwSession* q = static_cast<QwSession*>(s);
    ASR_REQUIRE(!q->aligner(), "qwen_decode: a forced-aligner session (classify_num %d) has no decode loop; call asr_qwen_align", q->cfg.classify_num);
    if (q->precision == ASR_PRECISION_BF16) q->step<bf16_t>(ids, next_ids_out, logits_out);
    else q->step<float>(ids, next_ids_out, logits_out);
  });
}

static QwSession* qwen_session(asr_session* s, const char* who) {
  ASR_REQUIRE(s && s->kind == 5, "%s: not a Qwen3-ASR session", who);
  return static_cast<QwSession*>(s);
}

extern "C" int asr_qwen_set_penalty(asr_session* s, float repeat_penalty, int penalty_range) {
  return asr_guard([&] { qwen_session(s, "qwen_set_penalty")->head.set_penalty(repeat_penalty, penalty_range, "qwen_set_penalty"); });
}

extern "C" int asr_qwen_track_history(asr_session* s, int enable) {
  return asr_guard([&] { qwen_session(s, "qwen_track_history")->head.set_track_history(enable != 0); });
}

extern "C" int asr_qwen_set_sampling(asr_session* s, int enable, float temperature, int top_k, float top_p, float repetition_penalty, uint64_t seed) {
  return asr_guard([&] {
// ... 90 lines not shown
```

### automatic-speech-recognition-asr-onnx_amd/csrc/sensevoice.hip

```cpp
#include <cstdlib>
#include <cstring>
#include <type_traits>

#include "../../include/asr_mi355x.h"
#include "engine.h"
#include "gemm.h"
#include "kernels.h"

namespace {

struct SvBlock {
  const float *ln1_g, *ln1_b, *bqkv, *wfsmn, *bfsmn, *ln2_g, *ln2_b, *b1, *b2;
  const float *cqkv, *c1;
  const void *wqkv, *wout, *w1, *w2;
  int in_size, kpad;
};

inline int round_up(int v, int m) { return (v + m - 1) / m * m; }

struct SvRunCtx;

struct PfDecLayer {
  const void *w1, *w2, *wq, *wkv, *wo;
  const float *b1, *b2, *n2_g, *n2_b, *wfsmn, *bq, *bkv, *bo;
  bool full;
};

struct SvSession : asr_session {
  bool paraformer = false;
  asr_paraformer_config pcfg{};
  std::vector<PfDecLayer> pdec;
  const void *cif_conv_w = nullptr, *pf_out_w = nullptr;
  const float *cif_conv_b = nullptr, *cif_out_w = nullptr, *cif_out_b = nullptr, *pf_out_b = nullptr;
  DeviceBuffer d_enc_lo, d_ck, d_cifa, d_alpha, d_dec, d_x2, d_sa, d_ffn32, d_tplan;
  DeviceBuffer d_wk_all, d_wv_all, d_bk_all, d_bv_all; int pf_n_full = 0; bool pf_kv_batch = true;
  template <typename T> void enqueue_paraformer_tail(const struct SvRunCtx& r);

  asr_sensevoice_config cfg;
  int feat = 0, kpad0 = 0, vpad = 0, max_lfr = 0;
  int n_bin_tiles = 0, n_kchunks = 0;
  std::vector<SvBlock> blocks;
  const float *dft = nullptr, *melp = nullptr, *cmvn_means = nullptr, *cmvn_vars = nullptr, *speech_pos = nullptr;
  const float *language_embed = nullptr, *system_embed = nullptr;
  const float *after_g = nullptr, *after_b = nullptr, *tp_g = nullptr, *tp_b = nullptr, *ctc_b = nullptr;
  const void* ctc_w = nullptr;

  DeviceBuffer d_ctplan, d_mdev, d_trow;
  DeviceBuffer d_sta, d_stb;
  DeviceBuffer d_x0lo, d_xalo, d_xblo;
  DeviceBuffer d_plan, d_audio, d_mel, d_x0, d_xa, d_xb, d_h, d_qk, d_vt, d_ctx, d_mem, d_ffn, d_amax_v, d_amax_i, d_ids,
      d_tok, d_num, d_logits;
  DeviceBuffer d_amax_s, d_flp, d_first, d_last, d_tlp;
  PinnedBuffer h_plan, h_out;

  int st_chunk = 0, st_B = 0, st_C = 0, st_en_cap = 0, st_de_cap = 0, st_max = 0, st_frames = 0;
  DeviceBuffer st_enk, st_env, st_dek, st_dev, st_defsmn, st_prev, st_cifh, st_cifa, st_enlen, st_delen, st_start, d_sqkv, d_skv;
  DeviceBuffer st_wpack, st_layer_tab, st_flags, st_times, st_dpack, st_dlayer_tab;
  bool st_dec_fused = false;
  int st_times_layer = -1;
  bool st_fused = false;
  int st_opt = 0;
  int st_fused_env = 2;
  int st_fused_max = 0, st_share_rule = 1, st_snapshot_env = -1, st_fault = 0, st_cooldown = 0;
  int st_giveups = 0, st_shared_steps = 0, st_snapshots = 0;
  static constexpr int st_cooldown_steps = 64;
  DeviceBuffer st_segs, st_shadow;
  int st_n_segs = 0, st_n_items = 0;
  void ensure_stream_shadow();
  void stream_init(int chunk, int look_back_encoder, int look_back_decoder, int max_streams);
  void stream_reset(int sid);
  template <typename T> void stream_step(const void* audio, int audio_mem, const int32_t* stream_ids, int n, int32_t* tok_out, int max_tokens,
                                         int32_t* num_out);
  bool use_graph = true;
  bool use_ln_alg = true;
  bool use_fused = true;
  bool use_block = true;
  bool use_fbank_split = true;
  DeviceBuffer d_dft_split;
  int block8_opt = 0;
  bool block_persist = true;
  DeviceBuffer d_layer_tab;
  bool use_tiles = true, tpack_ready = false;
  int tiles_opt = 0, tiles_dbg = -1;
  DeviceBuffer d_tpack, d_tlayer_tab, d_tkv;
  void ensure_tiles_pack();
  DeviceBuffer d_wpack;
  bool wpack_ready = false;
  void ensure_block_pack();
  int block_fault = 0;
  int block_giveups = 0;
  bool block_ffnk = true;
  bool foreign_now = false;
  int foreign_diverted = 0;
  int block_cooldown = 0;
  void load_env() {
    gemm_reload_env();
    if (const char* e = getenv("ASR_NO_GRAPH")) use_graph = !(e[0] == '1');
    if (const char* e = getenv("ASR_SANM_FUSED")) use_fused = !(e[0] == '0');
    if (const char* e = getenv("ASR_SANM_BLOCK")) use_block = !(e[0] == '0');
    if (const char* e = getenv("ASR_FBANK_SPLIT")) use_fbank_split = !(e[0] == '0');
    if (const char* e = getenv("ASR_SANM_BLOCK8_OPT")) block8_opt = atoi(e);
    if (const char* e = getenv("ASR_SANM_BLOCK_FFNK")) block_ffnk = !(e[0] == '0');
    if ((block8_opt >> 4) & 15) block_ffnk = false;
    if (const char* e = getenv("ASR_SANM_TILES")) use_tiles = !(e[0] == '0');
    if (const char* e = getenv("ASR_SANM_TILES_OPT")) tiles_opt = atoi(e);
    if (const char* e = getenv("ASR_SANM_TILES_DBG")) tiles_dbg = atoi(e);
    if (const char* e = getenv("ASR_SANM_BLOCK_PERSIST")) block_persist = !(e[0] == '0');
    if (const char* e = getenv("ASR_SANM_BLOCK_SCATTER")) block_scatter = e[0] == '1';
    if (const char* e = getenv("ASR_SANM_BLOCK_FAULT")) block_fault = e[0] == '1';
    if (const char* e = getenv("ASR_SANM_BLOCK_DBG")) block_dbg = atoi(e);
    if (const char* e = getenv("ASR_SANM_BLOCK_MIN")) block_min_utts = atoi(e);
    if (const char* e = getenv("ASR_LN_FUSED")) use_ln_alg = !(e[0] == '0');
  }
  int block_scatter = 0;
  int block_min_utts = 12;
  DeviceBuffer d_times; int block_dbg = -1;
  DeviceBuffer d_flags;
  StepGraph graph;
  uint64_t ws_epoch = 1;
  StepGraph st_graph[3];

  void init();
  void copy_block_status(const struct SvRunCtx& r);
  template <typename T> void enqueue(const struct SvRunCtx& r);
  template <typename T> void run(const void* audio, int audio_mem, const int64_t* offs, int batch, const int32_t* lang,
                                 int32_t* tok_out, int max_tokens, int32_t* num_out, int32_t* first_out = nullptr, int32_t* last_out = nullptr,
                                 float* logprob_out = nullptr);
  DeviceBuffer d_skws, d_skcnt;
  void gemm(const GemmArgs& g0) {
    if (!d_skws.ptr) { d_skws.reserve((size_t)16 << 20, stream); d_skcnt.reserve(4096 * 4, stream); }
    GemmArgs g = g0;
    g.sk_ws = d_skws.as<float>(); g.sk_ws_bytes = d_skws.cap; g.sk_cnt = d_skcnt.as<int32_t>();
    if (precision != ASR_PRECISION_BF16) { launch_gemm_f32(g, stream); return; }
    launch_gemm_bf16(g, stream);
  }
};

void SvSession::init() {
  const auto& c = cfg;
  ASR_REQUIRE(c.d_model == c.n_heads * c.d_head, "sensevoice: d_model != n_heads * d_head");
  ASR_REQUIRE(c.d_model % 128 == 0 && c.d_ffn % 128 == 0, "sensevoice: d_model and d_ffn must be multiples of 128");
  ASR_REQUIRE(c.d_head == 128 || (precision == ASR_PRECISION_F32 && c.d_head <= 128), "sensevoice: head_dim %d unsupported", c.d_head);
  ASR_REQUIRE(c.win_length == 400 && c.hop_length == 160, "sensevoice: front-end is built for 25 ms / 10 ms frames");
  ASR_REQUIRE(c.n_mels % 16 == 0, "sensevoice: n_mels must be a multiple of 16");
  ASR_REQUIRE(c.n_blocks >= 1 && c.n_main >= 1 && c.n_main <= c.n_blocks, "sensevoice: bad block counts");
  auto opt = [&](const std::string& n, std::initializer_list<int64_t> sh) -> const float* {
    return arena.has(n) ? (const float*)arena.get(n, ARENA_F32, sh).ptr : nullptr;
  };
  feat = c.n_mels * c.lfr_m;
  kpad0 = round_up(feat, 64);
  vpad = round_up(c.vocab, 128);
  n_bin_tiles = (c.nfft / 2 + 1 + 15) / 16;
  n_kchunks = c.win_length / 16;
  const int n_frames_max = (c.max_audio_len - c.win_length) / c.hop_length + 1;
  max_lfr = (n_frames_max + c.lfr_n - 1) / c.lfr_n;
  const int wt = precision == ASR_PRECISION_BF16 ? ARENA_BF16 : ARENA_F32;
  const int d = c.d_model, dff = c.d_ffn;

  dft = (const float*)arena.get("fe.dft", ARENA_F32, {(int64_t)n_bin_tiles * 2 * n_kchunks * 64 * 4}).ptr;
  if (precision == ASR_PRECISION_BF16 && use_fbank_split) {
    d_dft_split.reserve(fbank_split_table_bytes(n_bin_tiles, cfg.win_length), stream);
    launch_fbank_split_table(dft, n_bin_tiles, n_kchunks, d_dft_split.ptr, stream);
    HIP_CHECK(hipStreamSynchronize(stream));
  }
  melp = (const float*)arena.get("fe.mel", ARENA_F32, {(int64_t)(c.n_mels / 16) * n_bin_tiles * 64 * 4}).ptr;
  cmvn_means = opt("fe.cmvn_means", {feat});
  cmvn_vars = (const float*)arena.get("fe.cmvn_vars", ARENA_F32, {feat}).ptr;
  speech_pos = (const float*)arena.get("fe.speech_pos", ARENA_F32, {max_lfr, feat}).ptr;
  language_embed = c.n_prompt > 0 ? (const float*)arena.get("fe.language_embed", ARENA_F32, {c.n_languages, feat}).ptr : nullptr;
  system_embed = c.n_prompt > 1 ? (const float*)arena.get("fe.system_embed", ARENA_F32, {c.n_prompt - 1, feat}).ptr : nullptr;
  after_g = (const float*)arena.get("after_norm_g", ARENA_F32, {d}).ptr;
  after_b = (const float*)arena.get("after_norm_b", ARENA_F32, {d}).ptr;
  if (!paraformer) {
    tp_g = (const float*)arena.get("tp_norm_g", ARENA_F32, {d}).ptr;
    tp_b = (const float*)arena.get("tp_norm_b", ARENA_F32, {d}).ptr;
    ctc_w = arena.get("ctc.w", wt, {vpad, d}).ptr;
    ctc_b = (const float*)arena.get("ctc.b", ARENA_F32, {vpad}).ptr;
  } else {
    const int dd = pcfg.d_dec_ffn;
    ASR_REQUIRE(dd % 128 == 0 && dd <= 2048 && (3 * d) % 64 == 0 && pcfg.cif_kernel == 3, "paraformer: unsupported decoder geometry");
    cif_conv_w = arena.get("cif.conv_w", wt, {d, 3 * d}).ptr;
    cif_conv_b = (const float*)arena.get("cif.conv_b", ARENA_F32, {d}).ptr;
    cif_out_w = (const float*)arena.get("cif.out_w", ARENA_F32, {d}).ptr;
    cif_out_b = (const float*)arena.get("cif.out_b", ARENA_F32, {1}).ptr;
    pf_out_w = arena.get("out.w", wt, {vpad, d}).ptr;
    pf_out_b = (const float*)arena.get("out.b", ARENA_F32, {vpad}).ptr;
    pdec.resize(pcfg.n_dec + pcfg.n_dec3);
    for (int j = 0; j < (int)pdec.size(); ++j) {
      PfDecLayer& L = pdec[j];
      const std::string q = "dec" + std::to_string(j) + ".";
      L.full = j < pcfg.n_dec;
      L.w1 = arena.get(q + "w1", wt, {dd, d}).ptr;
      L.b1 = (const float*)arena.get(q + "b1", ARENA_F32, {dd}).ptr;
      L.w2 = arena.get(q + "w2", wt, {d, dd}).ptr;
      L.b2 = (const float*)arena.get(q + "b2", ARENA_F32, {d}).ptr;
      if (L.full) {
        L.n2_g = (const float*)arena.get(q + "n2_g", ARENA_F32, {d}).ptr;
        L.n2_b = (const float*)arena.get(q + "n2_b", ARENA_F32, {d}).ptr;
        L.wfsmn = (const float*)arena.get(q + "wfsmn", ARENA_F32, {d, c.fsmn_kernel}).ptr;
        L.wq = arena.get(q + "wq", wt, {d, d}).ptr;
        L.bq = (const float*)arena.get(q + "bq", ARENA_F32, {d}).ptr;
        L.wkv = arena.get(q + "wkv", wt, {2 * d, d}).ptr;
        L.bkv = (const float*)arena.get(q + "bkv", ARENA_F32, {2 * d}).ptr;
        L.wo = arena.get(q + "wo", wt, {d, d}).ptr;
        L.bo = (const float*)arena.get(q + "bo", ARENA_F32, {d}).ptr;
      }
    }
    if (const char* e = getenv("ASR_PF_KV_BATCH")) pf_kv_batch = !(e[0] == '0');
    pf_n_full = 0;
    for (const PfDecLayer& L : pdec) pf_n_full += L.full ? 1 : 0;
    if (pf_kv_batch && pf_n_full > 0) {
      const size_t ew = wt == ARENA_BF16 ? 2 : 4, wbytes = (size_t)d * d * ew;
      d_wk_all.reserve(pf_n_full * wbytes, stream); d_wv_all.reserve(pf_n_full * wbytes, stream);
      d_bk_all.reserve((size_t)pf_n_full * d * 4, stream); d_bv_all.reserve((size_t)pf_n_full * d * 4, stream);
      int li = 0;
      for (const PfDecLayer& L : pdec) {
        if (!L.full) continue;
        HIP_CHECK(hipMemcpyAsync((unsigned char*)d_wk_all.ptr + li * wbytes, L.wkv, wbytes, hipMemcpyDeviceToDevice, stream));
// ... 47 lines not shown
  for (int i = 0; i < cfg.n_blocks; ++i) {
    const SvBlock& b = blocks[i];
    if (b.in_size != cfg.d_model) continue;
    launch_sanm_block8_pack((const bf16_t*)b.wqkv, (const bf16_t*)b.wout, (const bf16_t*)b.w1, (const bf16_t*)b.w2, (unsigned char*)d_wpack.ptr + per * i, block_ffnk, stream);
  }
  std::vector<SanmBlockLayer> tab(cfg.n_blocks);
  for (int i = 0; i < cfg.n_blocks; ++i) {
    const SvBlock& b = blocks[i];
    tab[i] = SanmBlockLayer{b.bqkv, b.cqkv, b.wfsmn, b.bfsmn, b.b1, b.c1, b.b2, (const unsigned char*)d_wpack.ptr + per * i};
  }
  d_layer_tab.reserve(tab.size() * sizeof(SanmBlockLayer), stream);
  HIP_CHECK(hipMemcpyAsync(d_layer_tab.ptr, tab.data(), tab.size() * sizeof(SanmBlockLayer), hipMemcpyHostToDevice, stream));
  HIP_CHECK(hipStreamSynchronize(stream));
  wpack_ready = true;
}

void SvSession::copy_block_status(const SvRunCtx& r) {
  const size_t flag_words = (size_t)cfg.n_blocks * r.batch * 4;
  HIP_CHECK(hipMemcpyAsync(h_out.as<unsigned char>() + (size_t)r.batch * r.max_tokens * 4 + (size_t)r.batch * 4, d_flags.as<unsigned>() + flag_words, 4,
                           hipMemcpyDeviceToHost, stream));
}

void SvSession::ensure_tiles_pack() {
  if (tpack_ready) return;
  const size_t per = stream_layers_pack_bytes();
  d_tpack.reserve(per * cfg.n_blocks, stream);
  std::vector<StreamLayer> tab(cfg.n_blocks);
  for (int i = 0; i < cfg.n_blocks; ++i) {
    const SvBlock& b = blocks[i];
    tab[i] = StreamLayer{};
    if (b.in_size != cfg.d_model) continue;
    unsigned char* dst = (unsigned char*)d_tpack.ptr + per * i;
    launch_stream_layers_pack((const bf16_t*)b.wqkv, (const bf16_t*)b.wout, (const bf16_t*)b.w1, (const bf16_t*)b.w2, dst, stream);
    tab[i].wpack = dst; tab[i].bqkv = b.bqkv; tab[i].wfsmn = b.wfsmn; tab[i].bfsmn = b.bfsmn; tab[i].b1 = b.b1; tab[i].b2 = b.b2;
  }
  d_tlayer_tab.reserve(tab.size() * sizeof(StreamLayer), stream);
  HIP_CHECK(hipMemcpyAsync(d_tlayer_tab.ptr, tab.data(), tab.size() * sizeof(StreamLayer), hipMemcpyHostToDevice, stream));
  HIP_CHECK(hipStreamSynchronize(stream));
  tpack_ready = true;
}

template <typename T>
void SvSession::enqueue(const SvRunCtx& r) {
  const auto& c = cfg;
  const int d = c.d_model, dff = c.d_ffn, rows = r.rows, Mpad = r.Mpad;
  const int n_slabs = vpad / 64;
  {
    ProfScope ps(prof, "fbank", stream);
    FbankArgs fa;
    fa.audio = r.d_aud; fa.audio_dtype = audio_dtype; fa.plan = r.dp; fa.blk_utt = r.d_blk_utt; fa.blk_f0 = r.d_blk_f0;
    fa.dft_packed = dft; fa.mel_packed = melp; fa.mel_out = d_mel.as<float>();
    fa.n_bin_tiles = n_bin_tiles; fa.n_kchunks = n_kchunks; fa.n_mel_tiles = c.n_mels / 16; fa.n_mels = c.n_mels;
    fa.win = c.win_length; fa.hop = c.hop_length; fa.log_floor = 1.1920928955078125e-07f; fa.whisper = 0; fa.blk_max = nullptr;
    fa.dft_split = d_dft_split.ptr;
    launch_fbank(fa, r.n_fb, stream);
  }
  save_tap("mel", d_mel.ptr, r.frames, c.n_mels, c.n_mels, 4);
  bool alg = false;
  if constexpr (sizeof(T) == 2) {
    const SvBlock& b1 = blocks[c.n_blocks - 1];
    GemmArgs probe;
    probe.M = rows; probe.N = dff; probe.K = d; probe.ln_dim = d; probe.ln_colsum = b1.c1; probe.act = ACT_RELU; probe.bias = b1.b1;
    probe.out_lo = d_ffn.ptr; probe.A = d_xblo.ptr; probe.W = b1.w1;
    const bool skinny144 = gemm_skinny144_enabled();
    alg = (rows > 144 || !skinny144) && use_ln_alg && use_fused && b1.cqkv && b1.c1 && blocks[0].cqkv &&
          sanm_fused_supported(r.max_T, c.d_head, c.n_heads, d, c.fsmn_kernel, blocks[0].kpad) && gemm_ln_fusable(probe);
  }
  bf16_t* x0lo = d_x0lo.as<bf16_t>();
  bf16_t* xalo = d_xalo.as<bf16_t>();
  bf16_t* xblo = d_xblo.as<bf16_t>();
  {
    ProfScope ps(prof, "lfr_cmvn", stream);
    LfrArgs la;
    if (alg) la.out_lo = x0lo;
    la.mel = d_mel.as<float>(); la.plan = r.dp; la.row_utt = r.d_row_utt; la.cmvn_means = cmvn_means; la.cmvn_vars = cmvn_vars;
    la.speech_pos = speech_pos; la.language_embed = language_embed; la.system_embed = system_embed;
    la.out = d_x0.as<float>(); la.ld_out = kpad0; la.feat = feat; la.n_mels = c.n_mels; la.lfr_m = c.lfr_m; la.lfr_n = c.lfr_n;
    la.n_prompt = c.n_prompt; la.n_rows = Mpad; la.affine_mode = paraformer ? 1 : 0;
    launch_lfr_cmvn(la, stream);
  }
  save_tap("enc_in", d_x0.ptr, rows, feat, kpad0, 4);

  bool blk = false;
  if constexpr (sizeof(T) == 2)
    blk = use_block && block_cooldown == 0 && !foreign_now && use_ln_alg && use_fused && blocks[c.n_blocks - 1].cqkv && blocks[c.n_blocks - 1].c1 && c.n_blocks > 1 &&
          r.batch >= block_min_utts &&
          sanm_block_supported(r.max_T, c.d_head, c.n_heads, d, dff, c.fsmn_kernel);
  const size_t flag_words = (size_t)c.n_blocks * r.batch * 4;
  const size_t tile_flag0 = flag_words + 4 + (size_t)c.n_blocks * r.batch, tile_flag_stride = ((size_t)r.n_tiles + r.batch) * 4;
  const bool tiles = r.tiles && block_cooldown == 0 && !foreign_now;
  HIP_CHECK(hipMemsetAsync(d_flags.ptr, 0, (tile_flag0 + (tiles ? (size_t)c.n_blocks * tile_flag_stride : 0)) * 4, stream));
  const float* x_in = d_x0.as<float>();
  const bf16_t* x_in_lo = x0lo;
  const float2* st_in = nullptr;
  bool st_in_block8 = false;
  float2* sta = d_sta.as<float2>();
  float2* stb = d_stb.as<float2>();
  int ld_in = kpad0;
  float* xa = d_xa.as<float>();
  float* xb = d_xb.as<float>();
  T* h = d_h.as<T>();
  T* qk = d_qk.as<T>();
  T* vt = d_vt.as<T>();
  T* ctx = d_ctx.as<T>();
  float* mem = d_mem.as<float>();
  T* ffn = d_ffn.as<T>();
  for (int i = 0; i < c.n_blocks; ++i) {
// ... 736 lines not shown
  grow(d_qk, (size_t)Mpad * 2 * d * eT);
  grow(d_ctx, (size_t)Mpad * d * eT);
  grow(d_mem, (size_t)Mpad * d * 4);
  grow(d_ffn, (size_t)Mpad * std::max(dd, dff) * eT);
  grow(d_amax_v, (size_t)Mpad * n_slabs * 4);
  grow(d_amax_i, (size_t)Mpad * n_slabs * 4);
  grow(d_ids, (size_t)Mpad * 4);
  grow(d_tok, (size_t)n * max_tokens * 4);
  grow(d_num, (size_t)n * 4);
  grow(d_logits, (size_t)Mpad * vpad * 4);
  grow(d_enc_lo, (size_t)Mpad * d * eT);
  grow(d_cifa, (size_t)Mpad * 3 * d * eT);
  grow(d_alpha, (size_t)Mpad * 4);
  grow(d_dec, (size_t)Mpad * d * 4);
  grow(d_x2, (size_t)Mpad * d * 4);
  grow(d_sa, (size_t)Mpad * d * 4);
  grow(d_ffn32, (size_t)Mpad * dd * 4);
  grow(d_tplan, sizeof(UttPlan) * n);
  if (precision == ASR_PRECISION_BF16) {
    grow(d_xblo, (size_t)Mpad * d * 2);
    grow(d_stb, (size_t)Mpad * (d / 32) * 8);
  }
  const size_t out_bytes = (size_t)n * max_tokens * 4 + (size_t)n * 4;
  h_out.reserve(out_bytes + 16);
  HIP_CHECK(hipMemcpyAsync(d_plan.ptr, h_plan.ptr, plan_bytes, hipMemcpyHostToDevice, stream));
  const void* d_aud = audio;
  if (audio_mem == ASR_MEM_HOST) {
    HIP_CHECK(hipMemcpyAsync(d_audio.ptr, audio, (size_t)n * st_chunk * eA, hipMemcpyHostToDevice, stream));
    d_aud = d_audio.ptr;
  }
  bool step_fused = st_fused && std::is_same<T, bf16_t>::value && n <= st_fused_max && st_cooldown == 0 && !foreign_now;
  bool snapshot = false;
  if (st_cooldown > 0) --st_cooldown;
  if (step_fused && st_share_rule && asr_tenant_busy_others(this, 5.0) > 0) { step_fused = false; ++st_shared_steps; }
  if (step_fused) snapshot = st_snapshot_env == 1 || (st_snapshot_env < 0 && asr_tenant_live_others(this) > 0);
  if (snapshot) { ensure_stream_shadow(); ++st_snapshots; }
  const bool inject_fault = step_fused && st_fault == 1;
  if (inject_fault) st_fault = 2;
  const UttPlan* dp = d_plan.as<UttPlan>();
  const int32_t* d_blk_utt = (const int32_t*)((unsigned char*)d_plan.ptr + sizeof(UttPlan) * n);
  const int32_t* d_blk_f0 = d_blk_utt + n;
  const int32_t* d_row_utt = d_blk_f0 + n;

  auto enqueue = [&]() {
  if (snapshot && step_fused)
    launch_stream_state_copy(st_segs.as<StreamStateSeg>(), st_n_segs, st_n_items, dp, n, false, stream);
  {
    ProfScope ps(prof, "fbank", stream);
    FbankArgs fa;
    fa.audio = d_aud; fa.audio_dtype = audio_dtype; fa.plan = dp; fa.blk_utt = d_blk_utt; fa.blk_f0 = d_blk_f0;
    fa.dft_packed = dft; fa.mel_packed = melp; fa.mel_out = d_mel.as<float>();
    fa.n_bin_tiles = n_bin_tiles; fa.n_kchunks = n_kchunks; fa.n_mel_tiles = c.n_mels / 16; fa.n_mels = c.n_mels;
    fa.win = c.win_length; fa.hop = c.hop_length; fa.log_floor = 1.1920928955078125e-07f; fa.whisper = 0; fa.blk_max = nullptr;
    fa.dft_split = d_dft_split.ptr;
    launch_fbank(fa, n, stream);
  }
  if (taps_enabled) save_tap("mel", d_mel.ptr, frames, c.n_mels, c.n_mels, 4);
  {
    ProfScope ps(prof, "lfr_cmvn", stream);
    StreamLfrArgs la;
    la.mel = d_mel.as<float>(); la.plan = dp; la.cmvn_vars = cmvn_vars; la.pos_bias = speech_pos; la.prev = st_prev.as<float>();
    la.start = st_start.as<int32_t>(); la.out = d_x0.as<float>(); la.ld = kpad0; la.feat = feat; la.n_mels = c.n_mels; la.lfr_m = c.lfr_m;
    la.lfr_n = c.lfr_n; la.n_prev = st_C; la.n_new = st_B; la.n_rows = rows; la.n_frames = st_frames; la.pos_rows = max_lfr;
    launch_stream_lfr(la, stream);
    launch_stream_carry(d_x0.as<float>(), kpad0, dp, n, st_C, st_B, st_prev.as<float>(), st_start.as<int32_t>(), stream);
  }
  save_tap("enc_in", d_x0.ptr, rows, feat, kpad0, 4);
  const float* x_in = d_x0.as<float>();
  int ld_in = kpad0;
  float* xa = d_xa.as<float>();
  float* xb = d_xb.as<float>();
  T* h = d_h.as<T>();
  T* qkv = d_sqkv.as<T>();
  T* ctx = d_ctx.as<T>();
  float* mem = d_mem.as<float>();
  T* ffn = d_ffn.as<T>();
  const size_t en_layer = (size_t)st_max * H * st_en_cap * 128;
  const bool fused = step_fused;
  bool st_alg = false;
  bf16_t* xblo = nullptr;
  float2* stb = nullptr;
  if constexpr (sizeof(T) == 2) {
    const SvBlock& bl = blocks[c.n_blocks - 1];
    GemmArgs probe;
    probe.M = rows; probe.N = dff; probe.K = d; probe.ln_dim = d; probe.ln_colsum = bl.c1; probe.act = ACT_RELU; probe.bias = bl.b1;
    probe.out_lo = d_ffn.ptr; probe.A = d_xblo.ptr; probe.W = bl.w1;
    st_alg = use_ln_alg && bl.c1 && d_xblo.ptr && gemm_ln_fusable(probe);
    xblo = d_xblo.as<bf16_t>(); stb = d_stb.as<float2>();
  }
  for (int i = 0; i < c.n_blocks; ++i) {
    const SvBlock& b = blocks[i];
    if (fused && i == 1) {
      ProfScope ps(prof, "stream_layers", stream);
      const int nl = c.n_blocks - 1;
      HIP_CHECK(hipMemsetAsync(st_flags.ptr, 0, ((size_t)nl * n * 4 + 4 + (size_t)pdec.size() * n * 8) * 4, stream));
      StreamLayersArgs la;
      la.plan = dp; la.n_streams = n; la.n_layers = nl; la.n_cur = n_cur; la.cap = st_en_cap; la.roll_rows = st_B; la.ktaps = c.fsmn_kernel;
      la.ln_eps = 1e-5f; la.cache_len = st_enlen.as<int32_t>(); la.layers = st_layer_tab.as<StreamLayer>();
      la.x = xa; la.xb = xb; la.ctx = (bf16_t*)ctx; la.hid = (bf16_t*)ffn;
      la.flags = st_flags.as<unsigned>(); la.err = st_flags.as<unsigned>() + (size_t)nl * n * 4;
      la.opt = st_opt; la.fault = inject_fault ? 1 : 0;
      if (st_times_layer >= 0) {
        st_times.reserve((size_t)((n + 7) / 8) * 32 * 16 * 8, stream);
        HIP_CHECK(hipMemsetAsync(st_times.ptr, 0, (size_t)((n + 7) / 8) * 32 * 16 * 8, stream));
        la.times = st_times.as<unsigned long long>(); la.times_layer = st_times_layer;
      }
      launch_stream_layers(la, stream);
// ... 390 lines not shown
```

### automatic-speech-recognition-asr-onnx_amd/csrc/whisper.hip

```cpp
#include <cstdlib>
#include <cstring>

#include "../../include/asr_mi355x.h"
#include "decode_head.h"
#include "engine.h"
#include "gemm.h"
#include "kernels.h"

namespace {

inline int round_up(int v, int m) { return (v + m - 1) / m * m; }

template <typename T>
__global__ __launch_bounds__(256) void wh_beam_prompt_kernel(const T* __restrict__ pool, const int32_t* __restrict__ ptable, int pages_per_seq,
                                                             const T* __restrict__ kc, const T* __restrict__ vc, int max_pos, int B, int H, int p0, int beam,
                                                             int S, T* __restrict__ ext) {
  const int row = blockIdx.x, N = gridDim.x, lkh = blockIdx.y;
  const int h = lkh % H, kv = (lkh / H) & 1, l = lkh / (2 * H), b = row / beam;
  T* dst = ext + ((size_t)l * N + row) * 2 * H * S * 64 + ((size_t)kv * H + h) * S * 64;
  for (int i = threadIdx.x; i < p0 * 64; i += blockDim.x) {
    const int s = i >> 6, e = i & 63;
    const T* src = pool ? pool + (size_t)ptable[(size_t)b * pages_per_seq + (s >> 4)] * gridDim.y * 1024 + (size_t)lkh * 1024 + (size_t)(s & 15) * 64
                        : (kv ? vc : kc) + (((size_t)l * B + b) * H + h) * max_pos * 64 + (size_t)s * 64;
    dst[(size_t)s * 64 + e] = src[e];
  }
}

struct BeamStep {
  int beam = 1, p0 = 0, S = 0;
  const int32_t* src = nullptr; int ld_src = 0;
  int32_t* hist = nullptr;
  float* logits = nullptr;
};

struct EncLayer { const void *wqkv, *wo, *w1, *w2; const float *bqkv, *bo, *b1, *b2; };
struct DecLayer { const void *wqkv, *wo, *wcq, *wco, *w1, *w2; const float *bqkv, *bo, *bcq, *bco, *b1, *b2; };
struct Dec8Layer { const unsigned char* w[6]; const float* s[6]; const unsigned char* s4[6]; };
struct Enc8Layer { const unsigned char *w1, *w2; const float *s1, *s2; };

struct WhSession : asr_session {
  asr_whisper_config cfg;
  int vpad = 0, n_bin_tiles = 0, n_kchunks = 0, act = ACT_GELU_ERF;
  std::vector<EncLayer> enc;
  std::vector<DecLayer> dec;
  const float *dft = nullptr, *melp = nullptr, *conv1_b = nullptr, *conv2_b = nullptr, *enc_pos = nullptr, *enc_ln_g = nullptr,
              *enc_ln_b = nullptr, *ckv_b = nullptr, *dec_pos = nullptr, *suppress = nullptr, *begin = nullptr, *dec_ln_g = nullptr,
              *dec_ln_b = nullptr;
  const void *conv1_w = nullptr, *conv2_w = nullptr, *ckv_w = nullptr, *embed = nullptr;

  int batch = 0, rows = 0, Mpad = 0, hist = 0, max_T_enc = 0;
  std::vector<UttPlan> plan;
  DeviceBuffer d_plan, d_audio, d_mel, d_blkmax, d_x0, d_h1, d_xa, d_xb, d_xc, d_h, d_qk, d_vt, d_ctx, d_ffn, d_cross;
  DeviceBuffer d_kc, d_vc, d_ids, d_next, d_logits, d_dx, d_dqkv, d_dtok, d_hist;
  static constexpr int KV_PAGE = 16;
  DeviceBuffer d_kvpool, d_ptable;
  bool kv_paged = true;
  int kv_gens = 0, kv_batch = 0, kv_shuffle = 0;
  void ensure_kv_pages(int B, int positions, size_t elem_bytes);
  TokenHead head;
  DeviceBuffer d_nsp;
  bool use_graph = true;
  bool use_decode_gemm = true;
  DeviceBuffer d_colsum, d_dlo;
  bool fp8_mm = false;
  int fp8_act_shift = 0;
  std::vector<Enc8Layer> enc8;
  DeviceBuffer d_ew8, d_ewscale, d_h8, d_ffn8, d_sat;
  bool fp4 = false;
  bool fp8 = false, fp8_fake = false, fp8_weights = true, fp8_kv = true;
  std::vector<Dec8Layer> dec8;
  DeviceBuffer d_w8, d_wscale, d_wdq, d_cross8, d_cscale;
  StepGraph dec_graph;
  StepGraph beam_graph[2];
  DeviceBuffer d_bext, d_bhist, d_blogits;
  BeamRanker ranker;
  bool after_prefill = false;
  uint64_t ws_epoch = 1;
  PinnedBuffer h_plan, h_io;

  void init();
  DeviceBuffer d_skws, d_skcnt;
  static constexpr int SK_CNT = 4096;
  static constexpr size_t SK_WS_BYTES = (size_t)16 << 20;
  void gemm(const GemmArgs& g0) {
    if (precision != ASR_PRECISION_BF16) { launch_gemm_f32(g0, stream); return; }
    if (!d_skws.ptr) { d_skws.reserve(SK_WS_BYTES, stream); d_skcnt.reserve((size_t)SK_CNT * 4, stream); }
    GemmArgs g = g0;
    g.sk_ws = d_skws.as<float>(); g.sk_ws_bytes = SK_WS_BYTES; g.sk_cnt = d_skcnt.as<int32_t>();
    launch_gemm_bf16(g, stream);
  }
  template <typename T> void encode(const void* audio, int audio_mem, const int64_t* offs, int B, int32_t* n_pos_out);
  template <typename T> void enqueue_step(const int32_t* ids_dev, int n, bool is_prefill, bool use_hist_dev, const BeamStep* bs = nullptr);
  template <typename T> void step(const int32_t* ids_host, int n, bool is_prefill, int32_t* next_out, float* logits_out);
  template <typename T> void beam_search(int beam, int max_new, int eos_id, int32_t* tokens_out, int32_t* n_out, float* scores_out);
};

void WhSession::init() {
  const auto& c = cfg;
  ASR_REQUIRE(c.d_model == c.n_heads * c.d_head && c.d_head == 64, "whisper: head_dim must be 64 and d_model = heads * 64");
  ASR_REQUIRE(c.d_model % 128 == 0 && c.d_ffn % 128 == 0, "whisper: d_model and d_ffn must be multiples of 128");
  ASR_REQUIRE(c.nfft == 400 && c.hop_length == 160, "whisper: front-end is built for n_fft 400 / hop 160");
  ASR_REQUIRE(c.n_mels % 16 == 0 && (3 * c.n_mels) % 64 == 0, "whisper: n_mels must make 3*n_mels a multiple of 64");
  ASR_REQUIRE(c.max_target_positions <= 1536, "whisper: decoder context too long for the attention kernel");
  vpad = round_up(c.vocab, 128);
  head.init(c.max_target_positions, 0, 20, 512);
  n_bin_tiles = (c.nfft / 2 + 1 + 15) / 16;
  n_kchunks = c.nfft / 16;
  act = c.gelu_tanh ? ACT_GELU_TANH : ACT_GELU_ERF;
  const int wt = precision == ASR_PRECISION_BF16 ? ARENA_BF16 : ARENA_F32;
  const int d = c.d_model, dff = c.d_ffn, Ld = c.n_dec_layers;
  auto F = [&](const std::string& n, std::initializer_list<int64_t> sh) { return (const float*)arena.get(n, ARENA_F32, sh).ptr; };
  auto W = [&](const std::string& n, std::initializer_list<int64_t> sh) { return arena.get(n, wt, sh).ptr; };
  dft = F("fe.dft", {(int64_t)n_bin_tiles * 2 * n_kchunks * 64 * 4});
  melp = F("fe.mel", {(int64_t)(c.n_mels / 16) * n_bin_tiles * 64 * 4});
  conv1_w = W("enc.conv1_w", {d, 3 * c.n_mels});
  conv1_b = F("enc.conv1_b", {d});
  conv2_w = W("enc.conv2_w", {d, 3 * d});
  conv2_b = F("enc.conv2_b", {d});
  enc_pos = F("enc.pos", {c.max_source_positions, d});
  enc_ln_g = F("enc.ln_g", {d});
  enc_ln_b = F("enc.ln_b", {d});
  ckv_w = W("ckv.w", {2 * Ld * d, d});
  ckv_b = F("ckv.b", {2 * Ld * d});
  embed = W("dec.embed", {vpad, d});
  dec_pos = F("dec.pos", {c.max_target_positions, d});
  suppress = F("dec.suppress", {vpad});
  begin = F("dec.begin", {vpad});
  dec_ln_g = F("dec.ln_g", {d});
  dec_ln_b = F("dec.ln_b", {d});
  enc.resize(c.n_enc_layers);
  for (int i = 0; i < c.n_enc_layers; ++i) {
    const std::string p = "enc" + std::to_string(i) + ".";
    enc[i] = EncLayer{W(p + "wqkv", {3 * d, d}), W(p + "wo", {d, d}), W(p + "w1", {dff, d}), W(p + "w2", {d, dff}),
                      F(p + "bqkv", {3 * d}), F(p + "bo", {d}), F(p + "b1", {dff}), F(p + "b2", {d})};
  }
  dec.resize(Ld);
  for (int i = 0; i < Ld; ++i) {
    const std::string p = "dec" + std::to_string(i) + ".";
    dec[i] = DecLayer{W(p + "wqkv", {3 * d, d}), W(p + "wo", {d, d}), W(p + "wcq", {d, d}), W(p + "wco", {d, d}),
                      W(p + "w1", {dff, d}), W(p + "w2", {d, dff}),
                      F(p + "bqkv", {3 * d}), F(p + "bo", {d}), F(p + "bcq", {d}), F(p + "bco", {d}), F(p + "b1", {dff}), F(p + "b2", {d})};
  }
  if (fp8_mm) {
    ASR_REQUIRE(d % 256 == 0 && dff % 256 == 0, "whisper: FP8MM mode needs d_model and d_ffn to be multiples of 256");
    const size_t per = (size_t)2 * d * dff;
    d_ew8.reserve((size_t)c.n_enc_layers * per, stream); d_ewscale.reserve((size_t)c.n_enc_layers * (d + dff) * 4, stream);
    d_sat.reserve(8, stream); HIP_CHECK(hipMemsetAsync(d_sat.ptr, 0, 8, stream));
    enc8.resize(c.n_enc_layers);
    for (int i = 0; i < c.n_enc_layers; ++i) {
      unsigned char* w8 = d_ew8.as<unsigned char>() + i * per;
      float* sc = d_ewscale.as<float>() + (size_t)i * (d + dff);
      launch_quantize_rows_fp8((const bf16_t*)enc[i].w1, d, dff, d, w8, sc, nullptr, stream);
      launch_quantize_rows_fp8((const bf16_t*)enc[i].w2, dff, d, dff, w8 + (size_t)dff * d, sc + dff, nullptr, stream);
      enc8[i] = Enc8Layer{w8, w8 + (size_t)dff * d, sc, sc + dff};
    }
  }
  if (fp8 && fp8_weights) {
    ASR_REQUIRE(d % 256 == 0 && dff % 256 == 0, "whisper: FP8 / MXFP4 mode needs d_model and d_ffn to be multiples of 256");
    const size_t w_elems = (size_t)6 * d * d + (size_t)2 * d * dff, n_scales = (size_t)7 * d + dff;
    d_w8.reserve(fp4 ? Ld * w_elems / 2 : Ld * w_elems, stream); d_wscale.reserve(fp4 ? Ld * w_elems / 32 : Ld * n_scales * 4, stream); d_wdq.reserve(Ld * w_elems * 2, stream);
    dec8.resize(Ld);
    for (int i = 0; i < Ld; ++i) {
      DecLayer& L = dec[i];
      const void** slot[6] = {&L.wqkv, &L.wo, &L.wcq, &L.wco, &L.w1, &L.w2};
      const int Ns[6] = {3 * d, d, d, d, dff, d}, Ks[6] = {d, d, d, d, d, dff};
      unsigned char* w8 = d_w8.as<unsigned char>() + (fp4 ? i * w_elems / 2 : i * w_elems);
      bf16_t* dq = d_wdq.as<bf16_t>() + i * w_elems;
// ... 84 lines not shown
    for (int b = 0; b < B; ++b) {
      for (int f0 = 0; f0 < plan[b].n_frames; f0 += 64) { blk_utt[fi] = b; blk_f0[fi++] = f0; }
      for (int q0 = 0; q0 < plan[b].T; q0 += q_rows) { qb_utt[qi] = b; qb_q0[qi++] = q0; }
      const int rb = round_up(plan[b].T + 1, 16), rc = round_up(plan[b].T, 16);
      for (int t = 0; t < rc; ++t) row_utt[plan[b].row_off + t] = b;
      for (int t = 0; t < rb; ++t) {
        pos_rows[splan[b].row_off + t] = t < plan[b].T ? t : 0;
        grow_utt[2 * (splan[b].row_off + t)] = b;
        grow_utt[2 * (splan[b].row_off + t) + 1] = b;
      }
    }
  }
  { void* before = d_plan.ptr; d_plan.reserve(plan_bytes, stream); if (d_plan.ptr != before) ++ws_epoch; }
  HIP_CHECK(hipMemcpyAsync(d_plan.ptr, h_plan.ptr, plan_bytes, hipMemcpyHostToDevice, stream));
  const UttPlan* dp = d_plan.as<UttPlan>();
  const UttPlan* dps = dp + B;
  const int32_t* d_blk_utt = (const int32_t*)((unsigned char*)d_plan.ptr + 2 * sizeof(UttPlan) * B);
  const int32_t* d_blk_f0 = d_blk_utt + n_fb;
  const int32_t* d_qb_utt = d_blk_f0 + n_fb;
  const int32_t* d_qb_q0 = d_qb_utt + n_qb;
  const int32_t* d_row_utt = d_qb_q0 + n_qb;
  const int32_t* d_pos_rows = d_row_utt + Mpad;
  const int32_t* d_grow_utt = d_pos_rows + Mg;

  const size_t eT = sizeof(T);
  const size_t eA = audio_elt();
  const void* d_aud = static_cast<const unsigned char*>(audio) + (size_t)base0 * eA;
  if (audio_mem == ASR_MEM_HOST) {
    d_audio.reserve((size_t)total_samples * eA, stream);
    HIP_CHECK(hipMemcpyAsync(d_audio.ptr, d_aud, (size_t)total_samples * eA, hipMemcpyHostToDevice, stream));
    d_aud = d_audio.ptr;
  }
  const int Rpad = R + 256;
  d_mel.reserve((size_t)frames * c.n_mels * 4, stream);
  d_blkmax.reserve((size_t)n_fb * 4, stream);
  d_x0.reserve((size_t)(Rpad + 1) * c.n_mels * eT, stream);
  d_h1.reserve((size_t)Rpad * d * eT, stream);
  d_xa.reserve((size_t)Mpad * d * 4, stream);
  d_xb.reserve((size_t)Mpad * d * 4, stream);
  d_h.reserve((size_t)Mpad * d * eT, stream);
  d_qk.reserve((size_t)Mpad * 2 * d * eT, stream);
  d_vt.reserve((size_t)Mpad * d * eT, stream);
  d_ctx.reserve((size_t)Mpad * d * eT, stream);
  d_ffn.reserve(std::max((size_t)Mpad * dff * eT, (size_t)Mg * d * 4), stream);
  if (fp8_mm) { d_h8.reserve((size_t)Mpad * d, stream); d_ffn8.reserve((size_t)Mpad * dff, stream); }
  { void* before = d_cross.ptr; d_cross.reserve((size_t)2 * Ld * H * Mpad * 64 * eT, stream); if (d_cross.ptr != before) ++ws_epoch; }

  {
    ProfScope ps(prof, "logmel", stream);
    FbankArgs fa;
    fa.audio = d_aud; fa.audio_dtype = audio_dtype; fa.plan = dp; fa.blk_utt = d_blk_utt; fa.blk_f0 = d_blk_f0; fa.dft_packed = dft; fa.mel_packed = melp;
    fa.mel_out = d_mel.as<float>(); fa.n_bin_tiles = n_bin_tiles; fa.n_kchunks = n_kchunks; fa.n_mel_tiles = c.n_mels / 16;
    fa.n_mels = c.n_mels; fa.win = c.nfft; fa.hop = c.hop_length; fa.log_floor = 1e-10f; fa.whisper = 1;
    fa.blk_max = d_blkmax.as<float>();
    launch_fbank(fa, n_fb, stream);
    T* x0 = d_x0.as<T>();
    HIP_CHECK(hipMemsetAsync(x0, 0, (size_t)c.n_mels * eT, stream));
    launch_whisper_mel_finish<T>(d_mel.as<float>(), d_blkmax.as<float>(), dps, d_grow_utt, R, c.n_mels, x0 + c.n_mels, stream);
  }
  if (taps_enabled) save_tap("mel_gapped", d_x0.as<T>() + c.n_mels, R, c.n_mels, c.n_mels, (int)eT);
  {
    ProfScope ps(prof, "conv_stem", stream);
    GemmArgs g1;
    g1.A = d_x0.ptr; g1.lda = c.n_mels; g1.W = conv1_w; g1.ldw = 3 * c.n_mels; g1.M = R; g1.N = d; g1.K = 3 * c.n_mels;
    g1.bias = conv1_b; g1.act = act; g1.out_lo = d_h1.ptr; g1.ld_out_lo = d;
    gemm(g1);
    launch_zero_gap_rows<T>(d_h1.as<T>(), d, d, dps, d_grow_utt, R, stream);
    float* stem_out = d_ffn.as<float>();
    GemmArgs g2;
    g2.A = d_h1.ptr; g2.lda = 2 * d; g2.W = conv2_w; g2.ldw = 3 * d; g2.M = rows_g; g2.N = d; g2.K = 3 * d; g2.bias = conv2_b;
    g2.act = act; g2.add2 = enc_pos; g2.ld_add2 = d; g2.add2_rows = d_pos_rows; g2.out_f32 = stem_out; g2.ld_out_f32 = d;
    gemm(g2);
    launch_compact_rows(stem_out, dps, dp, d_row_utt, rows, d, d_xa.as<float>(), stream);
  }
  if (taps_enabled) save_tap("stem", d_xa.ptr, rows, d, d, 4);
  float* xa = d_xa.as<float>();
  float* xb = d_xb.as<float>();
  T* h = d_h.as<T>();
  T* qk = d_qk.as<T>();
  T* vt = d_vt.as<T>();
  T* ctx = d_ctx.as<T>();
  T* ffn = d_ffn.as<T>();
  for (int i = 0; i < c.n_enc_layers; ++i) {
    const EncLayer& L = enc[i];
    { ProfScope ps(prof, "layernorm", stream); launch_layernorm<T>(xa, d, rows, d, nullptr, nullptr, 1e-5f, h, d, d, stream); }
    {
      ProfScope ps(prof, "gemm_qkv", stream);
      GemmArgs g;
      g.A = h; g.lda = d; g.W = L.wqkv; g.ldw = d; g.M = rows; g.N = 2 * d; g.K = d; g.bias = L.bqkv; g.out_lo = qk; g.ld_out_lo = 2 * d;
      gemm(g);
      GemmArgs gv;
      gv.A = h; gv.lda = d; gv.W = (const T*)L.wqkv + (size_t)2 * d * d; gv.ldw = d; gv.M = rows; gv.N = d; gv.K = d;
      gv.bias = L.bqkv + 2 * d; gv.out_t = vt; gv.ld_out_t = Mpad;
      gemm(gv);
    }
    {
      ProfScope ps(prof, "attention", stream);
      AttnArgs aa;
      aa.q = qk; aa.k = qk + d; aa.ld_qk = 2 * d; aa.vt = vt; aa.ld_vt = Mpad; aa.ctx = ctx; aa.ld_ctx = d; aa.plan = dp;
      aa.qb_utt = d_qb_utt; aa.qb_q0 = d_qb_q0; aa.n_qblocks = n_qb; aa.n_heads = H; aa.qt = att_qt; aa.n_waves = att_nw; aa.max_T = max_T;
      if (precision == ASR_PRECISION_BF16) launch_attention_bf16_hd64(aa, stream);
      else launch_attention_f32(aa, c.d_head, stream);
    }
    {
      ProfScope ps(prof, "gemm_out", stream);
      GemmArgs g;
      g.A = ctx; g.lda = d; g.W = L.wo; g.ldw = d; g.M = rows; g.N = d; g.K = d; g.bias = L.bo; g.add = xa; g.ld_add = d;
// ... 342 lines not shown
  ranker.slots_dev = d_bhist.as<int32_t>(); ranker.slots_off = 1 - p0;
  if (max_new > 1) {
    const int P = (c.max_target_positions + KV_PAGE - 1) / KV_PAGE;
    const T* pool = kv_paged ? d_kvpool.as<T>() : nullptr;
    hipLaunchKernelGGL(wh_beam_prompt_kernel<T>, dim3(N, Ld * 2 * H), dim3(256), 0, stream, pool, kv_paged ? d_ptable.as<int32_t>() : nullptr, P,
                       kv_paged ? nullptr : d_kc.as<T>(), kv_paged ? nullptr : d_vc.as<T>(), c.max_target_positions, B, H, p0, beam, S, d_bext.as<T>());
    HIP_CHECK(hipGetLastError());
  }
  BeamStep bs;
  bs.beam = beam; bs.p0 = p0; bs.S = S; bs.ld_src = ld; bs.hist = d_bhist.as<int32_t>(); bs.logits = d_blogits.as<float>();
  const bool graphable = use_graph && !taps_enabled && !prof.enabled;
  GraphKey key;
  for (uint64_t v : {(uint64_t)B, (uint64_t)beam, (uint64_t)S, (uint64_t)p0, (uint64_t)ld, (uint64_t)n_stop, (uint64_t)Mpad, ws_epoch, ranker.epoch,
                     (uint64_t)(uintptr_t)stream})
    key.mix(v);
  for (int t = 0; t + 1 < max_new && !ranker.all_done(stream); ++t) {
    bs.src = ranker.ancestry();
    beam_graph[ranker.cur].run(stream, graphable, key.h, [&] { enqueue_step<T>(ranker.next_ids(), beam, false, true, &bs); });
    ranker.flip();
  }
  HIP_CHECK(hipGetLastError());
  ranker.download(tokens_out, max_new, n_out, scores_out, stream);
  if (prof.enabled) prof.collect();
}

}

extern "C" int asr_whisper_create(const asr_whisper_config* cfg, const void* arena, size_t arena_bytes, int arena_mem,
                                  int device_id, int precision, asr_session** out) {
  return asr_guard([&] {
    ASR_REQUIRE(cfg && arena && out, "whisper_create: null argument");
    ASR_REQUIRE(precision == ASR_PRECISION_BF16 || precision == ASR_PRECISION_F32 || precision == ASR_PRECISION_FP8W || precision == ASR_PRECISION_FP8MM ||
                precision == ASR_PRECISION_MXFP4W, "whisper_create: bad precision %d", precision);
    asr_require_device(device_id);
    WhSession* s = new WhSession();
    try {
      s->kind = 2;
      s->device = device_id;
      asr_tenant_attach(s);
      s->fp4 = precision == ASR_PRECISION_MXFP4W;
      s->fp8 = precision == ASR_PRECISION_FP8W || precision == ASR_PRECISION_FP8MM || s->fp4;
      s->fp8_mm = precision == ASR_PRECISION_FP8MM;
      s->precision = s->fp8 ? ASR_PRECISION_BF16 : precision;
      s->cfg = *cfg;
      gemm_reload_env();
      if (const char* e = getenv("ASR_FP8_FAKE")) s->fp8_fake = e[0] == '1';
      if (const char* e = getenv("ASR_FP8MM_ACT_SHIFT")) s->fp8_act_shift = std::min(std::max(atoi(e), 0), 16);
      if (const char* e = getenv("ASR_FP8_WEIGHTS")) s->fp8_weights = !(e[0] == '0');
      if (const char* e = getenv("ASR_FP8_KV")) s->fp8_kv = !(e[0] == '0');
      if (const char* e = getenv("ASR_NO_GRAPH")) s->use_graph = !(e[0] == '1');
      if (const char* e = getenv("ASR_KV_PAGED")) s->kv_paged = !(e[0] == '0');
      if (const char* e = getenv("ASR_KV_PAGE_SHUFFLE")) s->kv_shuffle = e[0] == '1';
      if (const char* e = getenv("ASR_DECODE_GEMM")) s->use_decode_gemm = !(e[0] == '0');
      HIP_CHECK(hipStreamCreateWithFlags(&s->stream, hipStreamNonBlocking));
      s->own_stream = true;
      s->arena.load(arena, arena_bytes, arena_mem, s->stream);
      s->init();
    } catch (...) {
      delete s;
      throw;
    }
    *out = s;
  });
}

extern "C" int asr_whisper_encode(asr_session* s, const void* audio, int audio_mem, const int64_t* audio_offsets, int batch,
                                  int32_t* n_positions_out) {
  return asr_guard([&] {
    ASR_REQUIRE(s && s->kind == 2, "whisper_encode: not a Whisper session");
    TenantScope tenant(s);
    WhSession* w = static_cast<WhSession*>(s);
    w->after_prefill = false;
    if (w->precision == ASR_PRECISION_BF16) w->encode<bf16_t>(audio, audio_mem, audio_offsets, batch, n_positions_out);
    else w->encode<float>(audio, audio_mem, audio_offsets, batch, n_positions_out);
  });
}

extern "C" int asr_whisper_prefill(asr_session* s, const int32_t* ids, int n, int32_t* next_ids_out, float* logits_out) {
  return asr_guard([&] {
    ASR_REQUIRE(s && s->kind == 2 && ids, "whisper_prefill: bad argument");
    TenantScope tenant(s);
    WhSession* w = static_cast<WhSession*>(s);
    w->after_prefill = false;
    if (w->precision == ASR_PRECISION_BF16) w->step<bf16_t>(ids, n, true, next_ids_out, logits_out);
    else w->step<float>(ids, n, true, next_ids_out, logits_out);
    w->after_prefill = true;
  });
}

extern "C" int asr_whisper_decode(asr_session* s, const int32_t* ids, int32_t* next_ids_out, float* logits_out) {
  return asr_guard([&] {
    ASR_REQUIRE(s && s->kind == 2, "whisper_decode: not a Whisper session");
    TenantScope tenant(s);
    WhSession* w = static_cast<WhSession*>(s);
    w->after_prefill = false;
    if (w->precision == ASR_PRECISION_BF16) w->step<bf16_t>(ids, 1, false, next_ids_out, logits_out);
    else w->step<float>(ids, 1, false, next_ids_out, logits_out);
  });
}

static WhSession* whisper_session(asr_session* s, const char* who) {
  ASR_REQUIRE(s && s->kind == 2, "%s: not a Whisper session", who);
  return static_cast<WhSession*>(s);
}

extern "C" int asr_whisper_set_penalty(asr_session* s, float repeat_penalty, int penalty_range) {
// ... 102 lines not shown
```

### include/asr_mi355x_probe.h

```cpp
#ifndef ASR_MI355X_PROBE_H
#define ASR_MI355X_PROBE_H
#include <stddef.h>
#include <stdint.h>
#ifdef __cplusplus
extern "C" {
#endif

typedef struct asr_probe_gemm_desc {
  int32_t M, N, K;
  const float* a;
  const float* w;
  const float* bias;
  const float* add;
  int32_t act;
  int32_t ln;
  float ln_eps;
  int32_t argmax;
  int32_t n_valid;
  int32_t variant;
  float* out_lo;
  float* out_f32;
  float* out_stats;
  int32_t* out_ids;
  char kernel[32];
// ... 47 lines not shown
  const int32_t* hist; const int32_t* T; const int32_t* row_off; const int32_t* row_seq; const int32_t* row_t;
  int32_t S_max;
  int32_t paged, n_pages, pps;
  const int32_t* table;
  int32_t hist_ld; const float* k_hist; const float* v_hist;
  int32_t after_ld; float* k_after; float* v_after;
  int32_t beam, ld_src, S_hyp;
  const int32_t* src; const int32_t* p0;
  float* ext_k; float* ext_v;
  float* q_out; float* k_rows_out; float* ctx;
  int32_t stray, qt, nw;
  char kernel[32];
} asr_probe_qwen_attn_desc;
int asr_probe_qwen_attention(asr_probe_qwen_attn_desc* d);

typedef struct asr_probe_beam_select_desc {
  int32_t n_utt, beam, K, ld, first, n_slots, n_stop;
  const float* topv; const int32_t* topi;
  float* cum; int32_t* fin; int32_t* len; int32_t* next; int32_t* done;
  const int32_t* stop;
  const int32_t* src_in; const int32_t* tok_in;
  int32_t* src_out; int32_t* tok_out;
} asr_probe_beam_select_desc;
int asr_probe_beam_select(asr_probe_beam_select_desc* d);

typedef struct asr_probe_token_head_desc {
  int32_t op, rows, n_valid, ld;
  float* logits;
  const float* vec;
  int32_t K;
  int32_t ld_save, n_saved;
  int32_t n_saved_after;
  int32_t* save_ids;
  int32_t range, partial;
  float value;
  const int32_t* next_in;
  float temperature, top_p, repetition_penalty;
  const float* noise;
  uint64_t seed;
  int32_t no_speech_id;
  float* out_v;
  int32_t* out_i;
  int32_t steps, track_history, sampling, change_step, range2;
  float value2;
  int32_t* picks;
} asr_probe_token_head_desc;
int asr_probe_token_head(asr_probe_token_head_desc* d);

int asr_probe_gemm_counts(int reset, char* buf, int cap);

int asr_probe_live_device_bytes(int64_t* bytes);

int asr_probe_gemm_bench(int variant, int M, int N, int K, int epilogue, int iters, float* avg_ms);
int asr_probe_grid_barrier(int n_workgroups, int iters, float* us_per_barrier);
int asr_probe_grid_barrier2(int n_workgroups, int iters, int mode, float* us_per_barrier);

#ifdef __cplusplus
}
#endif
#endif
```

Before: 77510 audio-s/s.

## Skip zero mel-filter bands in fbank and streamline CTC argmax epilogue

At session load, the packed mel filterbank is scanned on the host to find, for each mel tile, the range of frequency-bin tiles holding nonzero weights, plus the highest bin tile any filter uses. The fbank kernels then compute only the DFT bin tiles that are needed and run each mel tile's MFMA loop over its band only, with a register-resident path for narrow bands. Separately, the argmax/logsumexp GEMM epilogue precomputes bias values, uses v_max3 reductions and a min-index shuffle in place of paired value/index shuffles, and reuses the biased values for the exp-sum. The band tables are exact because only all-zero tiles are skipped, but they depend on the filter weights and cost one device-to-host sync at load time.

```diff
diff --git a/automatic-speech-recognition-asr-onnx_amd/_probe.py b/automatic-speech-recognition-asr-onnx_amd/_probe.py
--- a/automatic-speech-recognition-asr-onnx_amd/_probe.py
+++ b/automatic-speech-recognition-asr-onnx_amd/_probe.py
@@ -71,6 +71,7 @@
     "asr_probe_live_device_bytes": (C.c_int, [C.POINTER(C.c_int64)]),
     "asr_probe_gemm_fp8": (C.c_int, [C.c_int, C.c_int, C.c_int, C.c_void_p, C.c_void_p, _fp, C.c_float, _fp, _fp, C.c_int, C.c_void_p, _fp, C.c_int, _fp]),
     "asr_probe_gemm_bench": (C.c_int, [C.c_int] * 6 + [_fp]),
+    "asr_probe_fbank_bands": (C.c_int, [_fp, C.c_int, C.c_int, _ip, _ip, _ip]),
     "asr_probe_grid_barrier": (C.c_int, [C.c_int, C.c_int, _fp]),
     "asr_probe_grid_barrier2": (C.c_int, [C.c_int, C.c_int, C.c_int, _fp]),
 }
@@ -136,6 +137,15 @@
     ms = C.c_float(0.0)
     _lib.check(load().asr_probe_gemm_bench(variant, M, N, K, epilogue, iters, C.byref(ms)))
     return ms.value
+
+
+def fbank_bands(mel_packed, n_mel_tiles: int, n_bin_tiles: int):
+    m = _f32(mel_packed).reshape(-1)
+    assert m.size == n_mel_tiles * n_bin_tiles * 256, m.size
+    lo, hi = np.zeros(n_mel_tiles, np.int32), np.zeros(n_mel_tiles, np.int32)
+    n = C.c_int32(0)
+    _lib.check(load().asr_probe_fbank_bands(m.ctypes.data_as(_fp), n_mel_tiles, n_bin_tiles, lo.ctypes.data_as(_ip), hi.ctypes.data_as(_ip), C.byref(n)))
+    return [(int(a), int(b)) for a, b in zip(lo, hi)], n.value
 
 
 def gemm_set_variant(variant: int = -1) -> None:
diff --git a/automatic-speech-recognition-asr-onnx_amd/csrc/gemm_dev.h b/automatic-speech-recognition-asr-onnx_amd/csrc/gemm_dev.h
--- a/automatic-speech-recognition-asr-onnx_amd/csrc/gemm_dev.h
+++ b/automatic-speech-recognition-asr-onnx_amd/csrc/gemm_dev.h
@@ -78,6 +78,12 @@
   *reinterpret_cast<uint4*>(p) = w;
 }
 
+__device__ __forceinline__ float max3_f32(float a, float b, float c) {
+  float d;
+  asm("v_max3_f32 %0, %1, %2, %3" : "=v"(d) : "v"(a), "v"(b), "v"(c));
+  return d;
+}
+
 template <typename OutT, int ACT, int EPI, int NJ, int MI = 4>
 __device__ __forceinline__ void epilogue_rows(const GemmArgs& g, f32x4_t (&acc)[MI][NJ], int m_wave, int n_wave, int lane,
                                               const float2* ln_stats = nullptr,
@@ -88,26 +94,46 @@
   const bool want_f32 = epi_has<EPI, E_F32>(g.out_f32), want_lo = epi_has<EPI, E_LO>(g.out_lo);
   if (epi_has<EPI, E_AMAX>(g.amax_val)) {
     const int n_slabs = g.N / (NJ * 16), slab = n_wave / (NJ * 16);
+    const bool ragged = n_wave + NJ * 16 > g.n_valid;
+    constexpr int NONE = 1 << 20;
+    float bcol[NJ][4];
+#pragma unroll
+    for (int j = 0; j < NJ; ++j) {
+      const int n0 = n_wave + frag_col(j, fgrp * 4);
+#pragma unroll
+      for (int r = 0; r < 4; ++r) bcol[j][r] = has_bias ? (bias_at ? bias_at : g.bias)[n0 + r] : 0.0f;
+    }
 #pragma unroll
     for (int i = 0; i < MI; ++i) {
+      float v[NJ][4];
+#pragma unroll
+      for (int j = 0; j < NJ; ++j)
+#pragma unroll
+        for (int r = 0; r < 4; ++r) v[j][r] = acc[i][j][r] + bcol[j][r];
+      if (ragged) {
+#pragma unroll
+        for (int j = 0; j < NJ; ++j) {
+          const int n0 = n_wave + frag_col(j, fgrp * 4);
+#pragma unroll
+          for (int r = 0; r < 4; ++r)
+            if (n0 + r >= g.n_valid) v[j][r] = -INFINITY;
+        }
+      }
       float best = -INFINITY;
-      int bidx = 0x7fffffff;
-#pragma unroll
-      for (int j = 0; j < NJ; ++j) {
-        const int n0 = n_wave + frag_col(j, fgrp * 4);
-#pragma unroll
-        for (int r = 0; r < 4; ++r) {
-          float v = acc[i][j][r] + (has_bias ? (bias_at ? bias_at : g.bias)[n0 + r] : 0.0f);
-          if (n0 + r >= g.n_valid) v = -INFINITY;
-          if (v > best) { best = v; bidx = n0 + r; }
-        }
-      }
-#pragma unroll
-      for (int o = 16; o < 64; o <<= 1) {
-        const float ov = __shfl_xor(best, o, 64);
-        const int oi = __shfl_xor(bidx, o, 64);
-        if (ov > best || (ov == best && oi < bidx)) { best = ov; bidx = oi; }
-      }
+#pragma unroll
+      for (int j = 0; j < NJ; ++j) best = max3_f32(max3_f32(best, v[j][0], v[j][1]), v[j][2], v[j][3]);
+      best = fmaxf(best, __shfl_xor(best, 16, 64));
+      best = fmaxf(best, __shfl_xor(best, 32, 64));
+      int pos = NONE;
+#pragma unroll
+      for (int j = NJ - 1; j >= 0; --j)
+#pragma unroll
+        for (int r = 3; r >= 0; --r)
+          if (v[j][r] == best) pos = frag_col(j, 0) + r;
+      pos += fgrp * 8;
+      pos = min(pos, __shfl_xor(pos, 16, 64));
+      pos = min(pos, __shfl_xor(pos, 32, 64));
+      const int bidx = (pos >= NONE || !(best > -INFINITY)) ? 0x7fffffff : n_wave + pos;
       const int m = m_wave + i * 16 + frow;
       if (fgrp == 0 && m < g.M) {
         g.amax_val[(size_t)m * n_slabs + slab] = best;
@@ -117,15 +143,9 @@
         float sum = 0.0f;
         if (best != -INFINITY) {
 #pragma unroll
-          for (int j = 0; j < NJ; ++j) {
-            const int n0 = n_wave + frag_col(j, fgrp * 4);
-#pragma unroll
-            for (int r = 0; r < 4; ++r) {
-              float v = acc[i][j][r] + (has_bias ? (bias_at ? bias_at : g.bias)[n0 + r] : 0.0f);
-              if (n0 + r >= g.n_valid) v = -INFINITY;
-              sum += __expf(v - best);
-            }
-          }
+          for (int j = 0; j < NJ; ++j)
+#pragma unroll
+            for (int r = 0; r < 4; ++r) sum += __expf(v[j][r] - best);
         }
         sum += __shfl_xor(sum, 16, 64);
         sum += __shfl_xor(sum, 32, 64);
diff --git a/automatic-speech-recognition-asr-onnx_amd/csrc/kernels.h b/automatic-speech-recognition-asr-onnx_amd/csrc/kernels.h
--- a/automatic-speech-recognition-asr-onnx_amd/csrc/kernels.h
+++ b/automatic-speech-recognition-asr-onnx_amd/csrc/kernels.h
@@ -15,6 +15,14 @@
 
 enum { AUDIO_F32 = 0, AUDIO_I16 = 1, AUDIO_F16 = 2 };
 inline size_t audio_elt_bytes(int audio_dtype) { return audio_dtype == AUDIO_F32 ? 4 : 2; }
+constexpr int FB_MAX_MEL_TILES = 8;
+struct FbankBands {
+  uint8_t lo[FB_MAX_MEL_TILES] = {};
+  uint8_t hi[FB_MAX_MEL_TILES] = {};
+  int32_t n_dft_tiles = 0;
+};
+FbankBands fbank_bands(const float* mel_packed_dev, int n_mel_tiles, int n_bin_tiles, bool enabled, hipStream_t s);
+FbankBands fbank_bands_host(const float* mel_packed, int n_mel_tiles, int n_bin_tiles);
 struct FbankArgs {
   const void* audio;
   const UttPlan* plan;
@@ -34,6 +42,7 @@
   float* blk_max;
   const void* dft_split = nullptr;
   int audio_dtype = AUDIO_F32;
+  FbankBands bands;
 };
 void launch_fbank(const FbankArgs& a, int n_blocks, hipStream_t s);
 size_t fbank_split_table_bytes(int n_bin_tiles, int win);
diff --git a/automatic-speech-recognition-asr-onnx_amd/csrc/kernels.hip b/automatic-speech-recognition-asr-onnx_amd/csrc/kernels.hip
--- a/automatic-speech-recognition-asr-onnx_amd/csrc/kernels.hip
+++ b/automatic-speech-recognition-asr-onnx_amd/csrc/kernels.hip
@@ -2,6 +2,7 @@
 #include "gemm.h"
 
 #include <algorithm>
+#include <vector>
 #include <type_traits>
 #include <cstdlib>
 
@@ -33,6 +34,13 @@
   static __device__ __forceinline__ float widen(raw_t r, float) { return (float)__builtin_bit_cast(_Float16, (uint16_t)r); }
 };
 
+__device__ __forceinline__ int fb_band_lo(const FbankArgs& a, int nt) { return nt < FB_MAX_MEL_TILES ? a.bands.lo[nt] : 0; }
+__device__ __forceinline__ int fb_band_hi(const FbankArgs& a, int nt) {
+  const int h = nt < FB_MAX_MEL_TILES ? a.bands.hi[nt] : 0;
+  return h ? h : a.n_bin_tiles;
+}
+__device__ __forceinline__ int fb_dft_tiles(const FbankArgs& a) { return a.bands.n_dft_tiles ? a.bands.n_dft_tiles : a.n_bin_tiles; }
+
 template <typename S>
 __global__ __launch_bounds__(256) void fbank_kernel(const FbankArgs a) {
   extern __shared__ __attribute__((aligned(16))) unsigned char smem[];
@@ -68,7 +76,8 @@
 
   const int frow = lane & 15, fgrp = lane >> 4;
   const float4* dft = reinterpret_cast<const float4*>(a.dft_packed);
-  for (int t = wave; t < a.n_bin_tiles; t += 4) {
+  const int n_dft = fb_dft_tiles(a);
+  for (int t = wave; t < n_dft; t += 4) {
     f32x4_t re[4], im[4];
 #pragma unroll
     for (int mt = 0; mt < 4; ++mt) { re[mt] = f32x4_t{0.f, 0.f, 0.f, 0.f}; im[mt] = f32x4_t{0.f, 0.f, 0.f, 0.f}; }
@@ -107,10 +116,11 @@
   const float4* melp = reinterpret_cast<const float4*>(a.mel_packed);
   for (int nt = 0; nt < a.n_mel_tiles; ++nt) {
     f32x4_t acc = f32x4_t{0.f, 0.f, 0.f, 0.f};
-    float4 b4 = melp[(size_t)(nt * a.n_bin_tiles) * 64 + lane];
-    for (int kc = 0; kc < a.n_bin_tiles; ++kc) {
+    const int k_lo = fb_band_lo(a, nt), k_hi = fb_band_hi(a, nt);
+    float4 b4 = melp[(size_t)(nt * a.n_bin_tiles + k_lo) * 64 + lane];
+    for (int kc = k_lo; kc < k_hi; ++kc) {
       float4 b4n = b4;
-      if (kc + 1 < a.n_bin_tiles) b4n = melp[(size_t)(nt * a.n_bin_tiles + kc + 1) * 64 + lane];
+      if (kc + 1 < k_hi) b4n = melp[(size_t)(nt * a.n_bin_tiles + kc + 1) * 64 + lane];
       const float bv[4] = {b4.x, b4.y, b4.z, b4.w};
 #pragma unroll
       for (int j = 0; j < 4; ++j) {
@@ -192,7 +202,8 @@
   union BF { uint4 q; bf16x8_t v; };
   BF ring[FB_PF][6];
   const int wv = __builtin_amdgcn_readfirstlane(wave);
-  const int n_steps = (wv < a.n_bin_tiles && !(a.dbg & 1)) ? (a.n_bin_tiles - wv + FB_WAVES - 1) / FB_WAVES * FB_K32 : 0;
+  const int n_dft = fb_dft_tiles(a);
+  const int n_steps = (wv < n_dft && !(a.dbg & 1)) ? (n_dft - wv + FB_WAVES - 1) / FB_WAVES * FB_K32 : 0;
   constexpr size_t FB_IM = (size_t)FB_K32 * 3 * 64;
   auto frag_ptr = [&](int t, int kc) { return tab + (((size_t)(t * 2) * FB_K32 + kc) * 3) * 64 + lane; };
   int pt = wv, pkc = 0, ps = 0;
@@ -254,30 +265,65 @@
   float wmax = -INFINITY;
   const float4* melp = reinterpret_cast<const float4*>(a.mel_packed);
   constexpr int FB_MT = 4;
-  const int fw = wave & 3, mg = wave >> 2;
+  constexpr int FB_BAND = 8;
+  const int fw = wave & 3, mg = wv >> 2;
   for (int nt0 = mg; nt0 < ((a.dbg & 2) ? 0 : a.n_mel_tiles); nt0 += 2 * FB_MT) {
     f32x4_t acc[FB_MT];
-#pragma unroll
-    for (int q = 0; q < FB_MT; ++q) acc[q] = f32x4_t{0.f, 0.f, 0.f, 0.f};
-    auto mel_frags = [&](float4 (&b)[FB_MT], int kc) {
-#pragma unroll
-      for (int q = 0; q < FB_MT; ++q) b[q] = nt0 + 2 * q < a.n_mel_tiles ? melp[(size_t)((nt0 + 2 * q) * a.n_bin_tiles + kc) * 64 + lane] : make_float4(0.f, 0.f, 0.f, 0.f);
-    };
-    float4 b4[FB_MT], b4n[FB_MT];
-    mel_frags(b4, 0);
-    for (int kc = 0; kc < a.n_bin_tiles; ++kc) {
-      mel_frags(b4n, kc + 1 < a.n_bin_tiles ? kc + 1 : kc);
-#pragma unroll
-      for (int j = 0; j < 4; ++j) {
-        const float av = pw[(fw * 16 + frow) * FB_PLD + kc * 16 + j * 4 + fgrp];
+    int k_lo[FB_MT], k_hi[FB_MT], k_min = a.n_bin_tiles, k_max = 0;
+#pragma unroll
+    for (int q = 0; q < FB_MT; ++q) {
+      acc[q] = f32x4_t{0.f, 0.f, 0.f, 0.f};
+      const bool live = nt0 + 2 * q < a.n_mel_tiles;
+      k_lo[q] = live ? fb_band_lo(a, nt0 + 2 * q) : 0;
+      k_hi[q] = live ? fb_band_hi(a, nt0 + 2 * q) : 0;
+      if (live) { k_min = min(k_min, k_lo[q]); k_max = max(k_max, k_hi[q]); }
+    }
+    int len_max = 0;
+#pragma unroll
+    for (int q = 0; q < FB_MT; ++q) len_max = max(len_max, k_hi[q] - k_lo[q]);
+    const int pw_row = (fw * 16 + frow) * FB_PLD + fgrp;
+    if (len_max <= FB_BAND) {
+      float4 wq[FB_MT][FB_BAND];
+#pragma unroll
+      for (int q = 0; q < FB_MT; ++q) {
+        const int nt = min(nt0 + 2 * q, a.n_mel_tiles - 1);
+#pragma unroll
+        for (int i = 0; i < FB_BAND; ++i) wq[q][i] = melp[(size_t)(nt * a.n_bin_tiles + min(k_lo[q] + i, max(k_hi[q], 1) - 1)) * 64 + lane];
+      }
+#pragma unroll
+      for (int i = 0; i < FB_BAND; ++i) {
 #pragma unroll
         for (int q = 0; q < FB_MT; ++q) {
-          const float bv = j == 0 ? b4[q].x : j == 1 ? b4[q].y : j == 2 ? b4[q].z : b4[q].w;
-          if (nt0 + 2 * q < a.n_mel_tiles) acc[q] = __builtin_amdgcn_mfma_f32_16x16x4f32(av, bv, acc[q], 0, 0, 0);
+          if (k_lo[q] + i < k_hi[q]) {
+            const float* pr = pw + pw_row + (k_lo[q] + i) * 16;
+            acc[q] = __builtin_amdgcn_mfma_f32_16x16x4f32(pr[0], wq[q][i].x, acc[q], 0, 0, 0);
+            acc[q] = __builtin_amdgcn_mfma_f32_16x16x4f32(pr[4], wq[q][i].y, acc[q], 0, 0, 0);
+            acc[q] = __builtin_amdgcn_mfma_f32_16x16x4f32(pr[8], wq[q][i].z, acc[q], 0, 0, 0);
+            acc[q] = __builtin_amdgcn_mfma_f32_16x16x4f32(pr[12], wq[q][i].w, acc[q], 0, 0, 0);
+          }
         }
       }
-#pragma unroll
-      for (int q = 0; q < FB_MT; ++q) b4[q] = b4n[q];
+    } else {
+      auto mel_frags = [&](float4 (&b)[FB_MT], int kc) {
+#pragma unroll
+        for (int q = 0; q < FB_MT; ++q) b[q] = melp[(size_t)(min(nt0 + 2 * q, a.n_mel_tiles - 1) * a.n_bin_tiles + kc) * 64 + lane];
+      };
+      float4 b4[FB_MT], b4n[FB_MT];
+      mel_frags(b4, k_min);
+      for (int kc = k_min; kc < k_max; ++kc) {
+        mel_frags(b4n, kc + 1 < k_max ? kc + 1 : kc);
+#pragma unroll
+        for (int j = 0; j < 4; ++j) {
+          const float av = pw[pw_row + kc * 16 + j * 4];
+#pragma unroll
+          for (int q = 0; q < FB_MT; ++q) {
+            const float bv = j == 0 ? b4[q].x : j == 1 ? b4[q].y : j == 2 ? b4[q].z : b4[q].w;
+            if (kc >= k_lo[q] && kc < k_hi[q]) acc[q] = __builtin_amdgcn_mfma_f32_16x16x4f32(av, bv, acc[q], 0, 0, 0);
+          }
+        }
+#pragma unroll
+        for (int q = 0; q < FB_MT; ++q) b4[q] = b4n[q];
+      }
     }
 #pragma unroll
     for (int q = 0; q < FB_MT; ++q) {
@@ -1454,6 +1500,15 @@
   ASR_REQUIRE(a.win == WIN && a.hop == HOP, "fbank: only win=400 hop=160 is built (got %d/%d)", a.win, a.hop);
   ASR_REQUIRE(a.n_bin_tiles * 16 <= FB_PLD - 1, "fbank: too many frequency bins");
   ASR_REQUIRE(a.n_kchunks * 16 == WIN, "fbank: k-chunks must cover the window");
+  {
+    const int n_dft = a.bands.n_dft_tiles ? a.bands.n_dft_tiles : a.n_bin_tiles;
+    ASR_REQUIRE(n_dft >= 1 && n_dft <= a.n_bin_tiles, "fbank: band table computes %d of %d bin tiles", n_dft, a.n_bin_tiles);
+    for (int nt = 0; nt < std::min(a.n_mel_tiles, FB_MAX_MEL_TILES); ++nt) {
+      const int hi = a.bands.hi[nt] ? a.bands.hi[nt] : a.n_bin_tiles;
+      ASR_REQUIRE(a.bands.lo[nt] < hi && hi <= n_dft, "fbank: band [%d, %d) of mel tile %d does not fit %d computed bin tiles", (int)a.bands.lo[nt], hi, nt, n_dft);
+    }
+    ASR_REQUIRE(a.n_mel_tiles <= FB_MAX_MEL_TILES || a.bands.n_dft_tiles == 0, "fbank: a band table covers at most %d mel tiles", FB_MAX_MEL_TILES);
+  }
   const size_t lds = (size_t)(FB_AUDIO_LDS + FB_FRAMES * FB_PLD) * sizeof(float);
   static PerDeviceOnce attr_once;
   if (attr_once.first()) {
@@ -1481,6 +1536,34 @@
     case AUDIO_F16: return launch_fbank_typed<_Float16>(a, n_blocks, s);
     default: ASR_THROW(ASR_ERR_INVALID, "fbank: unknown audio sample type %d", a.audio_dtype);
   }
+}
+
+FbankBands fbank_bands_host(const float* mel_packed, int n_mel_tiles, int n_bin_tiles) {
+  FbankBands b;
+  if (n_mel_tiles > FB_MAX_MEL_TILES || n_bin_tiles > 255) return b;
+  int n_dft = 1;
+  for (int nt = 0; nt < n_mel_tiles; ++nt) {
+    int lo = n_bin_tiles, hi = 0;
+    for (int kc = 0; kc < n_bin_tiles; ++kc) {
+      const uint32_t* w = reinterpret_cast<const uint32_t*>(mel_packed) + (size_t)(nt * n_bin_tiles + kc) * 256;
+      bool any = false;
+      for (int i = 0; i < 256; ++i) any |= w[i] != 0u;
+      if (any) { lo = std::min(lo, kc); hi = kc + 1; }
+    }
+    if (hi == 0) { lo = 0; hi = 1; }
+    b.lo[nt] = (uint8_t)lo; b.hi[nt] = (uint8_t)hi;
+    n_dft = std::max(n_dft, hi);
+  }
+  b.n_dft_tiles = n_dft;
+  return b;
+}
+
+FbankBands fbank_bands(const float* mel_packed_dev, int n_mel_tiles, int n_bin_tiles, bool enabled, hipStream_t s) {
+  if (!enabled || n_mel_tiles > FB_MAX_MEL_TILES) return FbankBands{};
+  std::vector<float> h((size_t)n_mel_tiles * n_bin_tiles * 256);
+  HIP_CHECK(hipMemcpyAsync(h.data(), mel_packed_dev, h.size() * 4, hipMemcpyDeviceToHost, s));
+  HIP_CHECK(hipStreamSynchronize(s));
+  return fbank_bands_host(h.data(), n_mel_tiles, n_bin_tiles);
 }
 
 size_t fbank_split_table_bytes(int n_bin_tiles, int win) {
diff --git a/automatic-speech-recognition-asr-onnx_amd/csrc/probe.hip b/automatic-speech-recognition-asr-onnx_amd/csrc/probe.hip
--- a/automatic-speech-recognition-asr-onnx_amd/csrc/probe.hip
+++ b/automatic-speech-recognition-asr-onnx_amd/csrc/probe.hip
@@ -75,6 +75,13 @@
         g.out_lo = olo; g.ld_out_lo = N; g.st_out = st;
         break;
       }
+      case 8: {
+        ASR_REQUIRE(N % 64 == 0, "probe_gemm_bench: the arg-max head needs N %% 64 == 0");
+        g.amax_val = (float*)t.alloc((size_t)Mp * (N / 64) * 4);
+        g.amax_idx = (int32_t*)t.alloc((size_t)Mp * (N / 64) * 4);
+        g.n_valid = N;
+        break;
+      }
       default: ASR_THROW(ASR_ERR_INVALID, "probe_gemm_bench: unknown epilogue %d", epilogue);
     }
     g.dbg = variant < 0 ? 0 : variant >> 8;
@@ -108,6 +115,20 @@
   });
 }
 
+
+extern "C" int asr_probe_fbank_bands(const float* mel_packed, int n_mel_tiles, int n_bin_tiles, int32_t* lo, int32_t* hi, int32_t* n_dft_tiles) {
+  return asr_guard([&] {
+    ASR_REQUIRE(mel_packed && lo && hi && n_dft_tiles && n_mel_tiles > 0 && n_bin_tiles > 0, "probe_fbank_bands: bad argument");
+    asr_require_device(0);
+    Tmp t;
+    const size_t bytes = (size_t)n_mel_tiles * n_bin_tiles * 256 * 4;
+    float* d = (float*)t.alloc(bytes);
+    HIP_CHECK(hipMemcpy(d, mel_packed, bytes, hipMemcpyHostToDevice));
+    const FbankBands b = fbank_bands(d, n_mel_tiles, n_bin_tiles, true, nullptr);
+    for (int nt = 0; nt < n_mel_tiles; ++nt) { lo[nt] = nt < FB_MAX_MEL_TILES ? b.lo[nt] : 0; hi[nt] = nt < FB_MAX_MEL_TILES ? b.hi[nt] : 0; }
+    *n_dft_tiles = b.n_dft_tiles;
+  });
+}
 
 extern "C" int asr_probe_gemm_chain(int M, int N, int K, int epilogue, int cold_mb, int replays, float* us_per_launch) {
   return asr_guard([&] {
diff --git a/automatic-speech-recognition-asr-onnx_amd/csrc/qwen.hip b/automatic-speech-recognition-asr-onnx_amd/csrc/qwen.hip
--- a/automatic-speech-recognition-asr-onnx_amd/csrc/qwen.hip
+++ b/automatic-speech-recognition-asr-onnx_amd/csrc/qwen.hip
@@ -581,6 +581,8 @@
 struct QwSession : asr_session {
   asr_qwen_config cfg;
   int vpad = 0, hpad = 0, cpad = 0, n_bin_tiles = 0, n_kchunks = 0, chunk = 0, cpw = 0, rpw = 0, t_tok = 13;
+  bool use_fbank_bands = true;
+  FbankBands fb_bands;
   std::vector<QwEncLayer> enc;
   std::vector<QwDecLayer> dec;
   const float *dft = nullptr, *melp = nullptr, *conv1_b = nullptr, *conv2_b = nullptr, *conv3_b = nullptr, *enc_pos = nullptr,
@@ -666,6 +668,7 @@
   auto W = [&](const std::string& n, std::initializer_list<int64_t> sh) { return arena.get(n, wt, sh).ptr; };
   dft = F("fe.dft", {(int64_t)n_bin_tiles * 2 * n_kchunks * 64 * 4});
   melp = F("fe.mel", {(int64_t)(c.n_mels / 16) * n_bin_tiles * 64 * 4});
+  fb_bands = fbank_bands(melp, c.n_mels / 16, n_bin_tiles, use_fbank_bands, stream);
   conv1_w = W("enc.conv1_w", {cpad, 64});          conv1_b = F("enc.conv1_b", {cpad});
   conv2_w = W("enc.conv2_w", {cpad, 9 * cpad});    conv2_b = F("enc.conv2_b", {cpad});
   conv3_w = W("enc.conv3_w", {cpad, 9 * cpad});    conv3_b = F("enc.conv3_b", {cpad});
@@ -1104,7 +1107,7 @@
     FbankArgs fa;
     fa.audio = d_aud; fa.audio_dtype = audio_dtype; fa.plan = dup; fa.blk_utt = d_blk_utt; fa.blk_f0 = d_blk_f0; fa.dft_packed = dft; fa.mel_packed = melp;
     fa.mel_out = d_mel.as<float>(); fa.n_bin_tiles = n_bin_tiles; fa.n_kchunks = n_kchunks; fa.n_mel_tiles = c.n_mels / 16; fa.n_mels = c.n_mels;
-    fa.win = c.nfft; fa.hop = c.hop_length; fa.log_floor = 1e-10f; fa.whisper = 1; fa.blk_max = d_blkmax.as<float>();
+    fa.win = c.nfft; fa.hop = c.hop_length; fa.log_floor = 1e-10f; fa.whisper = 1; fa.blk_max = d_blkmax.as<float>(); fa.bands = fb_bands;
     launch_fbank(fa, n_fb, stream);
     if (taps_enabled) save_tap("mel", d_mel.ptr, frames, c.n_mels, c.n_mels, 4);
     hipLaunchKernelGGL(qw_mel_finish_kernel<T>, dim3(slots * chunk), dim3(128), 0, stream, d_mel.as<float>(), d_blkmax.as<float>(), dup, d_slot_utt,
@@ -1402,6 +1405,7 @@
       if (const char* e = getenv("ASR_QWEN_DECODE_GEMM")) s->use_decode_gemm = !(e[0] == '0');
       if (const char* e = getenv("ASR_NO_GRAPH")) s->use_graph = !(e[0] == '1');
       if (const char* e = getenv("ASR_QWEN_NO_FUSE")) s->no_fuse = e[0] == '1';
+      if (const char* e = getenv("ASR_FBANK_BANDS")) s->use_fbank_bands = !(e[0] == '0');
       if (const char* e = getenv("ASR_QWEN_KV_PAGED")) s->kv_paged = !(e[0] == '0');
       if (const char* e = getenv("ASR_KV_PAGE_SHUFFLE")) s->kv_shuffle = e[0] == '1';
       s->arena.load(arena, arena_bytes, arena_mem, s->stream);
diff --git a/automatic-speech-recognition-asr-onnx_amd/csrc/sensevoice.hip b/automatic-speech-recognition-asr-onnx_amd/csrc/sensevoice.hip
--- a/automatic-speech-recognition-asr-onnx_amd/csrc/sensevoice.hip
+++ b/automatic-speech-recognition-asr-onnx_amd/csrc/sensevoice.hip
@@ -76,6 +76,8 @@
   bool use_fused = true;
   bool use_block = true;
   bool use_fbank_split = true;
+  bool use_fbank_bands = true;
+  FbankBands fb_bands;
   DeviceBuffer d_dft_split;
   int block8_opt = 0;
   bool block_persist = true;
@@ -99,6 +101,7 @@
     if (const char* e = getenv("ASR_SANM_FUSED")) use_fused = !(e[0] == '0');
     if (const char* e = getenv("ASR_SANM_BLOCK")) use_block = !(e[0] == '0');
     if (const char* e = getenv("ASR_FBANK_SPLIT")) use_fbank_split = !(e[0] == '0');
+    if (const char* e = getenv("ASR_FBANK_BANDS")) use_fbank_bands = !(e[0] == '0');
     if (const char* e = getenv("ASR_SANM_BLOCK8_OPT")) block8_opt = atoi(e);
     if (const char* e = getenv("ASR_SANM_BLOCK_FFNK")) block_ffnk = !(e[0] == '0');
     if ((block8_opt >> 4) & 15) block_ffnk = false;
@@ -164,6 +167,7 @@
     HIP_CHECK(hipStreamSynchronize(stream));
   }
   melp = (const float*)arena.get("fe.mel", ARENA_F32, {(int64_t)(c.n_mels / 16) * n_bin_tiles * 64 * 4}).ptr;
+  fb_bands = fbank_bands(melp, c.n_mels / 16, n_bin_tiles, use_fbank_bands, stream);
   cmvn_means = opt("fe.cmvn_means", {feat});
   cmvn_vars = (const float*)arena.get("fe.cmvn_vars", ARENA_F32, {feat}).ptr;
   speech_pos = (const float*)arena.get("fe.speech_pos", ARENA_F32, {max_lfr, feat}).ptr;
@@ -317,7 +321,7 @@
     fa.dft_packed = dft; fa.mel_packed = melp; fa.mel_out = d_mel.as<float>();
     fa.n_bin_tiles = n_bin_tiles; fa.n_kchunks = n_kchunks; fa.n_mel_tiles = c.n_mels / 16; fa.n_mels = c.n_mels;
     fa.win = c.win_length; fa.hop = c.hop_length; fa.log_floor = 1.1920928955078125e-07f; fa.whisper = 0; fa.blk_max = nullptr;
-    fa.dft_split = d_dft_split.ptr;
+    fa.dft_split = d_dft_split.ptr; fa.bands = fb_bands;
     launch_fbank(fa, r.n_fb, stream);
   }
   save_tap("mel", d_mel.ptr, r.frames, c.n_mels, c.n_mels, 4);
@@ -1160,7 +1164,7 @@
     fa.dft_packed = dft; fa.mel_packed = melp; fa.mel_out = d_mel.as<float>();
     fa.n_bin_tiles = n_bin_tiles; fa.n_kchunks = n_kchunks; fa.n_mel_tiles = c.n_mels / 16; fa.n_mels = c.n_mels;
     fa.win = c.win_length; fa.hop = c.hop_length; fa.log_floor = 1.1920928955078125e-07f; fa.whisper = 0; fa.blk_max = nullptr;
-    fa.dft_split = d_dft_split.ptr;
+    fa.dft_split = d_dft_split.ptr; fa.bands = fb_bands;
     launch_fbank(fa, n, stream);
   }
   if (taps_enabled) save_tap("mel", d_mel.ptr, frames, c.n_mels, c.n_mels, 4);
diff --git a/automatic-speech-recognition-asr-onnx_amd/csrc/whisper.hip b/automatic-speech-recognition-asr-onnx_amd/csrc/whisper.hip
--- a/automatic-speech-recognition-asr-onnx_amd/csrc/whisper.hip
+++ b/automatic-speech-recognition-asr-onnx_amd/csrc/whisper.hip
@@ -41,6 +41,8 @@
 struct WhSession : asr_session {
   asr_whisper_config cfg;
   int vpad = 0, n_bin_tiles = 0, n_kchunks = 0, act = ACT_GELU_ERF;
+  bool use_fbank_bands = true;
+  FbankBands fb_bands;
   std::vector<EncLayer> enc;
   std::vector<DecLayer> dec;
   const float *dft = nullptr, *melp = nullptr, *conv1_b = nullptr, *conv2_b = nullptr, *enc_pos = nullptr, *enc_ln_g = nullptr,
@@ -113,6 +115,7 @@
   auto W = [&](const std::string& n, std::initializer_list<int64_t> sh) { return arena.get(n, wt, sh).ptr; };
   dft = F("fe.dft", {(int64_t)n_bin_tiles * 2 * n_kchunks * 64 * 4});
   melp = F("fe.mel", {(int64_t)(c.n_mels / 16) * n_bin_tiles * 64 * 4});
+  fb_bands = fbank_bands(melp, c.n_mels / 16, n_bin_tiles, use_fbank_bands, stream);
   conv1_w = W("enc.conv1_w", {d, 3 * c.n_mels});
   conv1_b = F("enc.conv1_b", {d});
   conv2_w = W("enc.conv2_w", {d, 3 * d});
@@ -303,7 +306,7 @@
     fa.audio = d_aud; fa.audio_dtype = audio_dtype; fa.plan = dp; fa.blk_utt = d_blk_utt; fa.blk_f0 = d_blk_f0; fa.dft_packed = dft; fa.mel_packed = melp;
     fa.mel_out = d_mel.as<float>(); fa.n_bin_tiles = n_bin_tiles; fa.n_kchunks = n_kchunks; fa.n_mel_tiles = c.n_mels / 16;
     fa.n_mels = c.n_mels; fa.win = c.nfft; fa.hop = c.hop_length; fa.log_floor = 1e-10f; fa.whisper = 1;
-    fa.blk_max = d_blkmax.as<float>();
+    fa.blk_max = d_blkmax.as<float>(); fa.bands = fb_bands;
     launch_fbank(fa, n_fb, stream);
     T* x0 = d_x0.as<T>();
     HIP_CHECK(hipMemsetAsync(x0, 0, (size_t)c.n_mels * eT, stream));
@@ -752,6 +755,7 @@
       if (const char* e = getenv("ASR_KV_PAGED")) s->kv_paged = !(e[0] == '0');
       if (const char* e = getenv("ASR_KV_PAGE_SHUFFLE")) s->kv_shuffle = e[0] == '1';
       if (const char* e = getenv("ASR_DECODE_GEMM")) s->use_decode_gemm = !(e[0] == '0');
+      if (const char* e = getenv("ASR_FBANK_BANDS")) s->use_fbank_bands = !(e[0] == '0');
       HIP_CHECK(hipStreamCreateWithFlags(&s->stream, hipStreamNonBlocking));
       s->own_stream = true;
       s->arena.load(arena, arena_bytes, arena_mem, s->stream);
diff --git a/include/asr_mi355x_probe.h b/include/asr_mi355x_probe.h
--- a/include/asr_mi355x_probe.h
+++ b/include/asr_mi355x_probe.h
@@ -123,6 +123,7 @@
 int asr_probe_live_device_bytes(int64_t* bytes);
 
 int asr_probe_gemm_bench(int variant, int M, int N, int K, int epilogue, int iters, float* avg_ms);
+int asr_probe_fbank_bands(const float* mel_packed, int n_mel_tiles, int n_bin_tiles, int32_t* lo, int32_t* hi, int32_t* n_dft_tiles);
 int asr_probe_grid_barrier(int n_workgroups, int iters, float* us_per_barrier);
 int asr_probe_grid_barrier2(int n_workgroups, int iters, int mode, float* us_per_barrier);
 
```

After: 78050 audio-s/s, median of 6. About the same (+0.7%).
